# mattayes/tigerbeetle

Measured on AMD Instinct MI355X. Metric: transfers/sec committed (whole node, bit-exact results) + p99 batch latency, higher is better.
Workload: dtype u128

## Files before the change

### tigerbeetle_amd/csrc/engine.hip

```cpp
#include <hip/hip_runtime.h>

#include <algorithm>
#include <atomic>
#include <chrono>
#include <cmath>
#include <cstdarg>
#include <cstdio>
#include <cstdlib>
#include <cstring>
#include <numeric>
#include <string>
#include <vector>
#include <map>
#include <functional>
#include <mutex>

#include "../../include/tbgpu.h"
#include "../../include/tbgpu_bench.h"
#include "../../include/tbgpu_shard.h"
#include "k_apply.h"
#include "k_flow.h"
#include "k_aux.h"
#include "k_replay.h"
#include "k_route.h"
// ... 306 lines not shown
    u64* h_rmeta = nullptr;
};

static inline BalView ckpt_view(const tbgpu* E) {
    return BalView{E->ckpt_bal, E->ckpt_bal ? E->ckpt_bal + 4 * E->account_cap : nullptr};
}

static void ckpt_note_ids(tbgpu* E, const u8* records, u64 n);

static int api_enter(tbgpu* E, bool mutates) {
    E->pf_input = nullptr;
    E->api_calls++;
    if (mutates && E->poisoned) {
        return fail(TBGPU_STATUS_PANIC, "engine stopped by an earlier device panic (tbgpu_reset or tbgpu_deinit it)");
    }
    return TBGPU_STATUS_OK;
}
#define API_ENTER(E, mutates)                        \
    do {                                             \
        if (const int st_ = api_enter((E), (mutates))) return st_; \
    } while (0)

static u64 pipe_reply_bytes(const tbgpu* E) { return 16 + E->meta_cap * 4 + (u64)E->pe_max * 8; }

#define PROF_EVENTS 8192

static int prof_begin(tbgpu* E, ProfilePair* p, int kind) {
    p->kind = -1;
    if (!E->profile || !(E->prof_mask & (1u << kind))) return 0;
    if (E->event_next + 2 > E->event_pool.size()) return 0;
    p->kind = kind;
    p->a = E->event_pool[E->event_next++];
    p->b = E->event_pool[E->event_next++];
    HIPCK(hipEventRecord(p->a, E->stream));
    return 0;
}

static int prof_end(tbgpu* E, ProfilePair* p) {
    if (!E->profile || p->kind < 0) return 0;
    HIPCK(hipEventRecord(p->b, E->stream));
    E->prof.push_back(*p);
    return 0;
}

static int prof_collect(tbgpu* E) {
    if (!E->kclock_used.empty()) {
        HIPCK(hipMemcpy(E->h_kclock, E->kclock, (u64)E->kclock_next * KCLOCK_WORDS * 8, hipMemcpyDeviceToHost));
        for (const auto& u : E->kclock_used) {
            const u64* w = E->h_kclock + (u64)u.first * KCLOCK_WORDS;
            for (u32 k = 0; k < 3; k++) {
                const u64* kw = w + k * KCLOCK_STRIDE;
                u64 end = 0;
                for (u32 q = 1; q <= KCLOCK_ENDS; q++) end = std::max(end, kw[q * KCLOCK_LINE]);
                if (k == 0) end = w[KCLOCK_STRIDE];
                if (!((u.second >> k) & 1) || end < kw[0] || !E->wall_khz) continue;
                E->span_ms[k] += (double)(end - kw[0]) / E->wall_khz;
                E->span_n[k] += 1;
            }
        }
        E->kclock_used.clear();
        E->kclock_next = 0;
    }
    for (const ProfilePair& p : E->prof) {
        float ms = 0;
        HIPCK(hipEventElapsedTime(&ms, p.a, p.b));
        E->prof_ms[p.kind] += ms;
        E->prof_n[p.kind] += 1;
        if (p.kind == K_PASS) E->pass_ms.push_back(ms);
    }
    E->prof.clear();
    E->event_next = 0;
    return 0;
}


static int engine_clear(tbgpu* E) {
    HIPCK(hipMemsetAsync(E->T.acct_hot, 0, E->account_cap * sizeof(AccountHot), E->stream));
    HIPCK(hipMemsetAsync(E->T.bal.lo, 0, E->account_cap * sizeof(AccountBal), E->stream));
    HIPCK(hipMemsetAsync(E->T.acct_cold, 0, E->account_cap * sizeof(AccountCold), E->stream));
    HIPCK(hipMemsetAsync(E->T.account_mark, 0, E->account_cap * sizeof(u32), E->stream));
    HIPCK(hipMemsetAsync(E->T.xidx, 0, E->xidx_cap * sizeof(u64), E->stream));
    HIPCK(hipMemsetAsync(E->T.xdup, 0, E->xidx_cap, E->stream));
    HIPCK(hipMemsetAsync(E->T.xposted, 0, E->xlog_cap, E->stream));
    HIPCK(hipMemsetAsync(E->bloom, 0, (E->bloom_mask + 1) / 8, E->stream));
    E->log_next = 0;
    E->evicted_total = 0;
    HIPCK(hipMemsetAsync(E->g, 0, sizeof(Globals), E->stream));
    HIPCK(hipStreamSynchronize(E->stream));
    E->epoch = 0;
    E->dedup_force = true;
    E->commit_ts = 0;
    E->last_batch_ts = 0;
    E->pending = false;
    E->balances_set = false;
    return TBGPU_STATUS_OK;
}

static std::mutex g_dev_mu;
static std::map<int, u32> g_dev_engines;

static void dev_register(tbgpu* E, bool add) {
    std::lock_guard<std::mutex> lock(g_dev_mu);
    if (add && !E->dev_registered) {
        g_dev_engines[E->device]++;
        E->dev_registered = true;
    } else if (!add && E->dev_registered) {
        if (--g_dev_engines[E->device] == 0) g_dev_engines.erase(E->device);
        E->dev_registered = false;
    }
}

__global__ __launch_bounds__(FLOW_THREADS) void tb_residency_probe(u32* counter, u32 total, u64 deadline, u32* failed) {
    extern __shared__ u32 s_probe_lds[];
    if (threadIdx.x != 0) return;
    s_probe_lds[0] = 0;
    atomicAdd(counter, 1u);
    const u64 t0 = wall_clock64();
    while (__hip_atomic_load(counter, __ATOMIC_RELAXED, __HIP_MEMORY_SCOPE_AGENT) < total) {
        if (wall_clock64() - t0 > deadline) {
            atomicOr(failed, 1u);
            return;
        }
        __builtin_amdgcn_s_sleep(8);
    }
}

static int residency_probe(tbgpu* E, u32 grid) {
    Owner scratch;
    u32* d = nullptr;
    HIPCK(tbMalloc(scratch, &d, 8));
    hipFuncAttributes attr{};
    size_t lds = 0;
    if (hipFuncGetAttributes(&attr, reinterpret_cast<const void*>(&tb_flow)) == hipSuccess) lds = attr.sharedSizeBytes;
    lds = std::max<size_t>(lds, 4);
    int probe_occ = 0;
    if (E->flow_occ &&
        hipOccupancyMaxActiveBlocksPerMultiprocessor(&probe_occ, reinterpret_cast<const void*>(&tb_residency_probe),
                                                     FLOW_THREADS, lds) == hipSuccess &&
        probe_occ > (int)E->flow_occ) {
        grid = (u32)(((u64)grid * (u64)probe_occ + E->flow_occ - 1) / E->flow_occ);
    }
    int st = TBGPU_STATUS_OK;
    u32 h[2] = {0, 0};
    hipError_t e = hipMemsetAsync(d, 0, 8, E->stream);
    if (e == hipSuccess) {
        hipLaunchKernelGGL(tb_residency_probe, dim3(grid), dim3(FLOW_THREADS), std::max<size_t>(lds, 4), E->stream, d, grid,
                           (u64)200 * E->wall_khz, d + 1);
        e = hipGetLastError();
    }
    if (e == hipSuccess) e = hipMemcpyAsync(h, d, 8, hipMemcpyDeviceToHost, E->stream);
    if (e == hipSuccess) e = hipStreamSynchronize(E->stream);
    if (e != hipSuccess) return fail(TBGPU_STATUS_DEVICE, "tbgpu_init: residency probe: %s", hipGetErrorString(e));
    if (h[1]) {
        st = fail(TBGPU_STATUS_DEVICE,
                  "tbgpu_init: device %d is not exclusive: %u workgroups of the ordered fallback's grid could not be "
                  "resident together (another process or kernel holds its CUs; tbgpu.h \"Device exclusivity\")",
                  E->device, grid);
    }
    return st;
}

static u32 flow_grid(tbgpu* E) {
    u32 engines = 1;
    {
        std::lock_guard<std::mutex> lock(g_dev_mu);
        auto it = g_dev_engines.find(E->device);
// ... 23 lines not shown
                                     tbgpu_delta_counts* counts);
static int node_api_get_stats(TbNode* N, tbgpu_stats* s);
static void node_reset_stats(TbNode* N);
static u32 node_world(TbNode* N);
static tbgpu* node_engine(TbNode* N, u32 d);
static int node_api_imports(TbNode* N, u32 d, u64 out[3]);
static int node_api_register_host(TbNode* N, void* ptr, u64 bytes);
static int node_api_unregister_host(TbNode* N, void* ptr);
static int node_fetch(TbNode* N, bool accounts, const u64* ids, u32 n, u8* out, u8* found);
static int node_api_accounts_in(TbNode* N, const void* records, u32 n, bool load);
static int node_api_transfers_in(TbNode* N, const void* records, const u8* state, u32 n, bool load);
static int node_api_set_commit_timestamp(TbNode* N, u64 timestamp);
static int query_init(tbgpu* E);
static void query_free(tbgpu* E);

static int engine_init(tbgpu* E);

extern "C" int tbgpu_init(const tbgpu_config* config, tbgpu_t** out) {
    *out = nullptr;
    if (config && config->device_count > 1) return node_api_init(config, out);
    if (!config || config->accounts_max == 0 || config->transfers_max == 0 || config->pass_events_max == 0 ||
        config->pass_batches_max == 0) {
        return fail(TBGPU_STATUS_INVALID, "tbgpu_init: invalid config");
    }
    if (config->accounts_max > (1ULL << 31) || config->transfers_max > (1ULL << 31)) {
        return fail(TBGPU_STATUS_INVALID, "tbgpu_init: table capacity above 2^31 objects per device");
    }
    int ndev = 0;
    if (hipGetDeviceCount(&ndev) != hipSuccess || ndev == 0) {
        return fail(TBGPU_STATUS_DEVICE, "tbgpu_init: no HIP device visible");
    }
    if (config->device < 0 || config->device >= ndev) {
        return fail(TBGPU_STATUS_INVALID, "tbgpu_init: device %d out of range (%d devices)", config->device, ndev);
    }
    tbgpu* E = new tbgpu();
    E->cfg = *config;
    E->device = config->device;
    E->profile = (config->flags & TBGPU_CONFIG_PROFILE) != 0;
#ifdef TBGPU_TIMING_KNOBS
    if (const char* ab = getenv("TBGPU_ABLATE")) E->ablate = (u32)strtoul(ab, nullptr, 0);
    E->kclock_off = getenv("TBGPU_NO_KCLOCK") != nullptr;
#endif
    const int st = engine_init(E);
    if (st) {
        tbgpu_deinit(E);
        return st;
    }
    *out = E;
    return TBGPU_STATUS_OK;
}

static int engine_init(tbgpu* E) {
    const tbgpu_config* config = &E->cfg;
    HIPCK(hipSetDevice(E->device));
    HIPCK(tbStreamCreate(E->own, &E->stream));
    dev_register(E, true);

    u64 load = 2;
#ifdef TBGPU_TIMING_KNOBS
    if (const char* s = getenv("TBGPU_ACCOUNT_SLOTS")) load = std::max<u64>(2, strtoull(s, nullptr, 0));
#endif
    E->account_cap = pow2_at_least(std::max<u64>(load * config->accounts_max, 1024));
    E->xlog_cap = std::max<u64>(config->transfers_max, 1024);
    E->xidx_cap = pow2_at_least(std::max<u64>(2 * E->xlog_cap, 2048));
    E->pe_max = config->pass_events_max;
    E->pb_max = config->pass_batches_max;
    if (const char* v = getenv("TBGPU_NO_LEAN")) E->lean_ok = atoi(v) == 0;
    if (const char* v = getenv("TBGPU_WB_BOUND")) E->wb_bound_ok = atoi(v) != 0;
    if (const char* v = getenv("TBGPU_WB_STAGE")) E->wb_stage = atoi(v) != 0;
    E->dedup_cap = pow2_at_least(std::max<u64>(4ULL * E->pe_max, 64));
    E->undo_cap = 4 * (BATCH_EVENTS_MAX + 1);
    E->meta_cap = std::max<u64>(E->pb_max, 1 << 16);
    E->lookup_cap = 1 << 16;
    {
        u32 shift = 0;
        while ((E->account_cap >> shift) > LEG_BUCKETS_PREF && (1u << shift) < LEG_SLOTS_MAX) shift++;
        E->leg_shift = shift;
        E->leg_buckets = (u32)(E->account_cap >> shift);
        E->legs_ok = E->leg_buckets <= LEG_BUCKETS_MAX;
    }

    size_t free_b = 0, total_b = 0;
    HIPCK(hipMemGetInfo(&free_b, &total_b));
    const u64 need = E->account_cap * (sizeof(Account) + 4) + E->xlog_cap * (sizeof(Transfer) + 1) +
                     E->xidx_cap * (sizeof(u64) + 1) +
                     (u64)E->pe_max * (4 * 4 + 8 * 4 + 128 * PIPE_SLOTS + 8 + 4) + E->dedup_cap * 8;
    if (need > free_b) {
        return fail(TBGPU_STATUS_INVALID, "tbgpu_init: needs %llu bytes of HBM, %llu free",
                    (unsigned long long)need, (unsigned long long)free_b);
    }

    HIPCK(tbMalloc(E->own, &E->T.acct_hot, E->account_cap * sizeof(AccountHot)));
    HIPCK(tbMalloc(E->own, &E->T.bal.lo, E->account_cap * sizeof(AccountBal)));
    E->T.bal.hi = E->T.bal.lo + 4 * E->account_cap;
    HIPCK(tbMalloc(E->own, &E->T.acct_cold, E->account_cap * sizeof(AccountCold)));
    HIPCK(tbMalloc(E->own, &E->T.account_mark, E->account_cap * sizeof(u32)));
    HIPCK(tbMalloc(E->own, &E->T.xidx, E->xidx_cap * sizeof(u64)));
    HIPCK(tbMalloc(E->own, &E->T.xdup, E->xidx_cap));
    HIPCK(tbMalloc(E->own, &E->T.xlog, E->xlog_cap * sizeof(Transfer)));
    HIPCK(tbMalloc(E->own, &E->T.xposted, E->xlog_cap));
    HIPCK(tbMalloc(E->own, &E->g, sizeof(Globals)));
    {
        const u64 bits = std::min<u64>(1ULL << 34, pow2_at_least(std::max<u64>(1ULL << 16, 8 * E->xlog_cap)));
        E->bloom_mask = bits - 1;
        HIPCK(tbMalloc(E->own, &E->bloom, bits / 8));
    }
    {
        hipDeviceProp_t prop;
        int occ = 0;
        if (hipGetDeviceProperties(&prop, E->device) == hipSuccess &&
            hipOccupancyMaxActiveBlocksPerMultiprocessor(&occ, reinterpret_cast<const void*>(&tb_flow), FLOW_THREADS, 0) ==
                hipSuccess &&
            occ >= 1) {
            E->F.grid = (u32)std::max(1, std::min(prop.multiProcessorCount / 4, 64));
#ifdef TBGPU_TIMING_KNOBS
            if (const char* gs = getenv("TBGPU_FLOW_GRID")) E->F.grid = std::max(1u, std::min(E->F.grid, (u32)atoi(gs)));
#endif
            E->flow_capacity = (u64)occ * prop.multiProcessorCount;
            E->flow_occ = (u32)occ;
            E->F.grid = (u32)std::min<u64>(E->F.grid, E->flow_capacity);
            E->F.grid_alloc = E->F.grid;
            int khz = 0;
            if (hipDeviceGetAttribute(&khz, hipDeviceAttributeWallClockRate, E->device) != hipSuccess) khz = 0;
            khz = std::max(khz, 100000);
            E->F.stall_ticks = 60ULL * 1000ULL * (u64)khz;
            if (const char* ms = getenv("TBGPU_STALL_MS")) {
                E->F.stall_ticks = std::max<u64>(1, strtoull(ms, nullptr, 10)) * (u64)khz;
            }
            E->wall_khz = (u64)khz;
            if (getenv("TBGPU_DEBUG")) {
                fprintf(stderr, "tbgpu: flow grid %u, occupancy %d, wall clock %d kHz, stall ticks %llu\n", E->F.grid,
                        occ, khz, (unsigned long long)E->F.stall_ticks);
            }
            E->flow_ok = E->pb_max <= FLOW_NB_MAX && !(config->flags & TBGPU_CONFIG_SEQUENTIAL_FALLBACK);
#ifdef TBGPU_TIMING_KNOBS
            if (getenv("TBGPU_NO_FLOW")) E->flow_ok = false;
#endif
        }
    }
    E->T.account_mask = E->account_cap - 1;
    E->T.xidx_mask = E->xidx_cap - 1;
    E->T.xlog_cap = E->xlog_cap;
    E->T.g = E->g;

    const u64 pe = E->pe_max;
    HIPCK(tbMalloc(E->own, &E->info, pe * 4));
    HIPCK(tbMalloc(E->own, &E->eflags, pe * 2));
    HIPCK(tbMalloc(E->own, &E->dr, pe * 4));
    HIPCK(tbMalloc(E->own, &E->cr, pe * 4));
    HIPCK(tbMalloc(E->own, &E->ps, pe * 4));
    HIPCK(tbMalloc(E->own, &E->rs, pe * 4));
    HIPCK(tbMalloc(E->own, &E->dep_list, pe * 4));
    HIPCK(tbMalloc(E->own, &E->dep_count, (u64)E->pb_max * 4));
    HIPCK(tbMalloc(E->own, &E->amt, pe * 16));
    HIPCK(tbMalloc(E->own, &E->kid, pe * 8));
    HIPCK(tbMalloc(E->own, &E->kpid, pe * 8));
    HIPCK(tbMalloc(E->own, &E->dedup, E->dedup_cap * 8));
    HIPCK(tbMalloc(E->own, &E->sum_shards, SUM_WORDS * 8));
    HIPCK(tbMalloc(E->own, &E->undo, (u64)E->undo_cap * sizeof(UndoEntry)));
    if (E->legs_ok) {
        HIPCK(tbMalloc(E->own, &E->resolve_slow, (u64)E->pb_max * 4));
        HIPCK(tbMalloc(E->own, &E->leg_w, pe * 2 * 8));
        HIPCK(tbMalloc(E->own, &E->leg_off, (u64)std::min<u32>(E->pb_max, LEG_PREPARES_MAX) * (E->leg_buckets + 1) * 4));
        HIPCK(tbMalloc(E->own, &E->leg_tot, ((u64)E->leg_buckets + 1) * 4));
        HIPCK(hipMemset(E->leg_tot, 0, ((u64)E->leg_buckets + 1) * 4));
    }
    if (E->flow_ok) {
        FlowArgs& F = E->F;
        HIPCK(tbMalloc(E->own, &F.f_pe, pe * 4));
        HIPCK(tbMalloc(E->own, &F.f_batch, pe * 4));
        HIPCK(tbMalloc(E->own, &F.f_len, pe * 4));
        HIPCK(tbMalloc(E->own, &F.need, pe * 4));
        HIPCK(tbMalloc(E->own, &F.nsucc, pe * 4));
        HIPCK(tbMalloc(E->own, &F.queue, pe * 4));
        HIPCK(tbMalloc(E->own, &F.uflags, pe * 4));
        HIPCK(tbMalloc(E->own, &F.nacct, pe * 4));
        HIPCK(tbMalloc(E->own, &F.rpos, pe * 4));
        HIPCK(tbMalloc(E->own, &F.succ, pe * 4 * FLOW_RMAX));
        HIPCK(tbMalloc(E->own, &F.run, pe * sizeof(RunEntry) * FLOW_RMAX));
        for (int k = 0; k < 2; k++) {
            HIPCK(tbMalloc(E->own, &F.keys[k], pe * 4 * FLOW_RMAX));
            HIPCK(tbMalloc(E->own, &F.vals[k], pe * 4 * FLOW_RMAX));
        }
// ... 2178 lines not shown
extern "C" int tbgpu_load_accounts(tbgpu_t* E, const void* records, uint32_t n) {
    API_ENTER(E, true);
    if (E->node) return node_api_accounts_in(E->node, records, n, true);
    return upsert_accounts(E, records, n, true);
}

static int upsert_transfers(tbgpu* E, const void* records, const uint8_t* state, uint32_t n, bool if_absent) {
    HIPCK(hipSetDevice(E->device));
    if (if_absent) {
        if (E->pending) {
            int st = engine_sync(E);
            if (st) return st;
        }
        int st = load_snapshot(E, records, n);
        if (st) return st;
    }
    if (E->pending) {
        int st = engine_sync(E);
        if (st) return st;
    }
    HIPCK(hipMemsetAsync(E->d_status, 0, 8, E->stream));
    for (u32 c = 0; c < n; c += E->lookup_cap) {
        const u32 m = std::min<u32>(E->lookup_cap, n - c);
        HIPCK(hipMemcpyAsync(E->lookup_out, (const u8*)records + (u64)c * 128, (u64)m * 128, hipMemcpyHostToDevice,
                             E->stream));
        HIPCK(hipMemcpyAsync(E->lookup_found, state + c, m, hipMemcpyHostToDevice, E->stream));
        HIPCK(hipMemsetAsync(E->d_status + 1, 0, 4, E->stream));
        hipLaunchKernelGGL(tb_upsert_transfers, dim3((m + 255) / 256), dim3(256), 0, E->stream, E->T, E->lookup_out,
                           E->lookup_found, m, E->log_next, E->d_status + 1, E->d_status, if_absent ? 1u : 0u,
                           nullptr);
        HIPCK(hipGetLastError());
        u32 added = 0;
        HIPCK(hipMemcpyAsync(&added, E->d_status + 1, 4, hipMemcpyDeviceToHost, E->stream));
        HIPCK(hipStreamSynchronize(E->stream));
        E->log_next += added;
    }
    u32 status = 0;
    HIPCK(hipMemcpy(&status, E->d_status, 4, hipMemcpyDeviceToHost));
    if (status) return fail(TBGPU_STATUS_PANIC, "transfer log or index full");
    return TBGPU_STATUS_OK;
}

extern "C" int tbgpu_upsert_transfers(tbgpu_t* E, const void* records, const uint8_t* state, uint32_t n) {
    API_ENTER(E, true);
    if (E->node) return node_api_transfers_in(E->node, records, state, n, false);
    return upsert_transfers(E, records, state, n, false);
}

extern "C" int tbgpu_load_transfers(tbgpu_t* E, const void* records, const uint8_t* posted_state, uint32_t n) {
    API_ENTER(E, true);
    if (E->node) return node_api_transfers_in(E->node, records, posted_state, n, true);
    std::vector<u8> st(n);
    for (u32 i = 0; i < n; i++) {
        if (posted_state[i] > POSTED_VOIDED) return fail(TBGPU_STATUS_INVALID, "posted state %u", posted_state[i]);
        st[i] = (u8)(posted_state[i] + 1);
    }
    return upsert_transfers(E, records, st.data(), n, true);
}

static int engine_evict(tbgpu_t* E, uint64_t keep, uint64_t* evicted) {
    *evicted = 0;
    HIPCK(hipSetDevice(E->device));
    if (E->wb.inflight) return fail(TBGPU_STATUS_INVALID, "an asynchronous write-back is in flight");
    int st = engine_sync(E);
    if (st) return st;
    if (E->ckpt_valid && E->ckpt_pos != E->log_next)
        return fail(TBGPU_STATUS_INVALID, "%llu log positions written since the last write-back",
                    (unsigned long long)(E->log_next - E->ckpt_pos));
    const u64 written = E->ckpt_valid ? E->ckpt_pos : 0;
    const u64 cut = std::min<u64>(written, E->log_next > keep ? E->log_next - keep : 0);
    if (cut == 0) return TBGPU_STATUS_OK;
    const u64 n = E->log_next, kept = n - cut;
    u8* live = E->T.xdup;
    u64* d_evicted = E->wb.d_cnt;
    HIPCK(hipMemsetAsync(d_evicted, 0, 8, E->stream));
    const u32 grid = (u32)std::min<u64>(4096, std::max<u64>(1, (n + 255) / 256));
    hipLaunchKernelGGL(tb_evict_scan, dim3(grid), dim3(256), 0, E->stream, E->T, cut, n, E->bloom, E->bloom_mask, live,
                       d_evicted);
    HIPCK(hipGetLastError());
    for (u64 a = 0; a < kept; a += cut) {
        const u64 m = std::min<u64>(cut, kept - a);
        HIPCK(hipMemcpyAsync(E->T.xlog + a, E->T.xlog + cut + a, m * sizeof(Transfer), hipMemcpyDeviceToDevice, E->stream));
        HIPCK(hipMemcpyAsync(E->T.xposted + a, E->T.xposted + cut + a, m, hipMemcpyDeviceToDevice, E->stream));
    }
    HIPCK(hipMemsetAsync(E->T.xlog + kept, 0, cut * sizeof(Transfer), E->stream));
    HIPCK(hipMemsetAsync(E->T.xposted + kept, 0, cut, E->stream));
    HIPCK(hipMemsetAsync(E->T.xidx, 0, E->xidx_cap * sizeof(u64), E->stream));
    if (kept) {
        hipLaunchKernelGGL(tb_evict_reindex, dim3((u32)std::min<u64>(4096, (kept + 255) / 256)), dim3(256), 0, E->stream,
                           E->T, kept, (const u8*)live);
        HIPCK(hipGetLastError());
    }
    HIPCK(hipMemsetAsync(E->T.xdup, 0, E->xidx_cap, E->stream));
    u64 h_evicted = 0;
    HIPCK(hipMemcpyAsync(&h_evicted, d_evicted, 8, hipMemcpyDeviceToHost, E->stream));
    HIPCK(hipStreamSynchronize(E->stream));
    E->log_next = kept;
    E->ckpt_pos -= cut;
    E->evicted_total += h_evicted;
    E->dedup_force = true;
    if (h_evicted) {
        HIPCK(hipMemcpy(E->h_globals, E->g, sizeof(Globals), hipMemcpyDeviceToHost));
        E->h_globals->transfer_count -= std::min<u64>(E->h_globals->transfer_count, h_evicted);
        HIPCK(hipMemcpy(&E->g->transfer_count, &E->h_globals->transfer_count, 8, hipMemcpyHostToDevice));
    }
    *evicted = h_evicted;
    return TBGPU_STATUS_OK;
}


extern "C" int tbgpu_evict_transfers(tbgpu_t* E, uint64_t keep, uint64_t* evicted) {
    API_ENTER(E, true);
    *evicted = 0;
    if (E->node) return node_api_evict(E->node, keep, evicted);
    return engine_evict(E, keep, evicted);
}

static int engine_maybe_cold(tbgpu_t* E, const uint64_t* ids, uint32_t n, uint8_t* cold) {
    if (n == 0) return TBGPU_STATUS_OK;
    if (E->evicted_total == 0) {
        memset(cold, 0, n);
        return TBGPU_STATUS_OK;
    }
    HIPCK(hipSetDevice(E->device));
    if (E->pending) {
        const int st = engine_sync(E);
        if (st) return st;
    }
    for (u32 i0 = 0; i0 < n; i0 += E->lookup_cap) {
        const u32 m = std::min<u32>(n - i0, E->lookup_cap);
        HIPCK(hipMemcpyAsync(E->lookup_ids, ids + 2 * (u64)i0, (u64)m * 16, hipMemcpyHostToDevice, E->stream));
        hipLaunchKernelGGL(tb_cold_query, dim3((m + 255) / 256), dim3(256), 0, E->stream, E->T, (const u64*)E->bloom,
                           E->bloom_mask, E->lookup_ids, m, E->lookup_found);
        HIPCK(hipGetLastError());
        HIPCK(hipMemcpyAsync(cold + i0, E->lookup_found, m, hipMemcpyDeviceToHost, E->stream));
        HIPCK(hipStreamSynchronize(E->stream));
    }
    return TBGPU_STATUS_OK;
}

extern "C" int tbgpu_transfers_maybe_cold(tbgpu_t* E, const uint64_t* ids, uint32_t n, uint8_t* cold) {
    API_ENTER(E, false);
    if (E->node) return node_api_maybe_cold(E->node, ids, n, cold);
    return engine_maybe_cold(E, ids, n, cold);
}

extern "C" int tbgpu_set_commit_timestamp(tbgpu_t* E, uint64_t timestamp) {
    API_ENTER(E, true);
    if (E->node) return node_api_set_commit_timestamp(E->node, timestamp);
    HIPCK(hipSetDevice(E->device));
    if (E->pending) {
        int st = engine_sync(E);
        if (st) return st;
    }
    E->commit_ts = timestamp;
    E->last_batch_ts = timestamp;
    HIPCK(hipMemcpyAsync(&E->g->commit_timestamp, &E->commit_ts, 8, hipMemcpyHostToDevice, E->stream));
    HIPCK(hipStreamSynchronize(E->stream));
    return TBGPU_STATUS_OK;
}

#include "query.h"
#include "node.h"
```

### tigerbeetle_amd/csrc/k_aux.h

```cpp
#pragma once

#include "pass.h"

template <bool ACCOUNTS>
__global__ void tb_lookup(Tables T, const u64* ids, u32 n, u8* out, u8* found) {
    const u32 i = blockIdx.x * blockDim.x + threadIdx.x;
    if (i >= n) return;
    const u64 lo = ids[2 * i], hi = ids[2 * i + 1];
    if (ACCOUNTS) {
        const u32 slot = tb_account_find(T, lo, hi);
        found[i] = slot != TB_NOT_FOUND;
        if (slot != TB_NOT_FOUND) *(Account*)(out + (u64)i * 128) = tb_account_load(T, slot);
    } else {
        const u32 pos = tb_transfer_find(T, lo, hi);
        found[i] = pos != TB_NOT_FOUND;
        if (pos != TB_NOT_FOUND) *(Transfer*)(out + (u64)i * 128) = T.xlog[pos];
    }
}

__global__ void tb_export_accounts(Tables T, u64 first, u64 cap, u8* out, u64* count) {
    const u64 i = first + (u64)blockIdx.x * blockDim.x + threadIdx.x;
    if (i >= cap) return;
    const AccountHot& h = T.acct_hot[i];
    if (h.timestamp == 0 || tb_id_reserved(h.id_lo, h.id_hi)) return;
    const u64 k = atomicAdd((unsigned long long*)count, 1ULL);
    *(Account*)(out + k * 128) = tb_account_load(T, (u32)i);
}

__global__ void tb_export_transfers(Tables T, u64 first, u64 n, u8* out, u64* count, u64* posted_out,
                                    u64* posted_count) {
    const u64 i = first + (u64)blockIdx.x * blockDim.x + threadIdx.x;
    if (i >= first + n) return;
    const u64 e = T.xidx[i];
    if (e == 0 || (e & XI_TOMB)) return;
    const u32 pos = tb_xi_pos(e);
    const Transfer& t = T.xlog[pos];
    const u64 k = atomicAdd((unsigned long long*)count, 1ULL);
    *(Transfer*)(out + k * 128) = t;
    const u8 st = T.xposted[pos];
    if (st != POSTED_NONE) {
        const u64 q = atomicAdd((unsigned long long*)posted_count, 1ULL);
        posted_out[2 * q] = t.timestamp;
        posted_out[2 * q + 1] = st == POSTED_POSTED ? 0 : 1;
    }
}

__global__ void tb_set_balances(Tables T, u64 lo, u64 hi, u64 dp_lo, u64 dp_hi, u64 dpo_lo, u64 dpo_hi,
                                u64 cp_lo, u64 cp_hi, u64 cpo_lo, u64 cpo_hi, u32* status) {
    const u32 slot = tb_account_find(T, lo, hi);
    if (slot == TB_NOT_FOUND) {
        *status = 1;
        return;
    }
    AccountBal a;
    a.debits_pending = tb_u128(dp_lo, dp_hi);
    a.debits_posted = tb_u128(dpo_lo, dpo_hi);
    a.credits_pending = tb_u128(cp_lo, cp_hi);
    a.credits_posted = tb_u128(cpo_lo, cpo_hi);
    tb_bal_store(T.bal, slot, a);
    const u128 d = tb_sat_add(a.debits_pending, a.debits_posted);
    const u128 c = tb_sat_add(a.credits_pending, a.credits_posted);
    u128 bound = tb_u128(T.g->bound_lo, T.g->bound_hi);
    if (d > bound) bound = d;
    if (c > bound) bound = c;
    T.g->bound_lo = tb_lo(bound);
    T.g->bound_hi = tb_hi(bound);
    *status = 0;
}

__global__ void tb_zero_balances(Tables T, u64 cap) {
    const u64 i = (u64)blockIdx.x * blockDim.x + threadIdx.x;
    if (i == 0) {
        T.g->transfer_count = 0;
        T.g->bound_lo = 0;
        T.g->bound_hi = 0;
    }
    if (i >= cap) return;
    tb_bal_store(T.bal, i, AccountBal{0, 0, 0, 0});
}

__global__ void tb_delta_accounts(Tables T, BalView snap, u64 ts0, u64 first, u64 last, u8* out, u64 cap,
                                  u64* count, AccountBal* before, u32 world, u32 self) {
    const u64 i = first + (u64)blockIdx.x * blockDim.x + threadIdx.x;
    if (i >= last) return;
    const AccountHot& h = T.acct_hot[i];
    if (h.timestamp == 0 || tb_id_reserved(h.id_lo, h.id_hi)) return;
    if (world > 1 && tb_home(h.id_lo, h.id_hi, world) != self) return;
    const AccountBal b = tb_bal_load(T.bal, i), s = tb_bal_load(snap, i);
    const bool same = b.debits_pending == s.debits_pending && b.debits_posted == s.debits_posted &&
                      b.credits_pending == s.credits_pending && b.credits_posted == s.credits_posted;
    if (h.timestamp <= ts0 && same) return;
    const u64 k = atomicAdd((unsigned long long*)count, 1ULL);
    if (k < cap) {
        *(Account*)(out + k * 128) = tb_account_load(T, (u32)i);
        if (before) before[k] = h.timestamp <= ts0 ? s : AccountBal{0, 0, 0, 0};
    }
}

#define DELTA_THREADS 256

__device__ static inline bool tb_delta_live(const Tables& T, u64 pos, u64 ts0) {
    const Transfer& t = T.xlog[pos];
    return t.timestamp > ts0 && tb_transfer_find(T, tb_lo(t.id), tb_hi(t.id)) == (u32)pos;
}

__global__ __launch_bounds__(DELTA_THREADS) void tb_delta_log_count(Tables T, u64 pos0, u64 n, u64 ts0, u32* block_counts) {
    __shared__ u32 s_wave[DELTA_THREADS / 64];
    const u64 i = (u64)blockIdx.x * DELTA_THREADS + threadIdx.x;
    const bool live = i < n && tb_delta_live(T, pos0 + i, ts0);
    const u64 m = __ballot(live);
    if ((threadIdx.x & 63) == 0) s_wave[threadIdx.x >> 6] = __popcll(m);
    __syncthreads();
    if (threadIdx.x == 0) {
        u32 c = 0;
        for (u32 w = 0; w < DELTA_THREADS / 64; w++) c += s_wave[w];
        block_counts[blockIdx.x] = c;
    }
}

__global__ __launch_bounds__(DELTA_THREADS) void tb_delta_log_scatter(Tables T, u64 pos0, u64 n, u64 ts0, const u64* block_base,
                                                                      u8* out, u64* ids, u64* pv, u64* pv_count) {
    __shared__ u32 s_wave[DELTA_THREADS / 64];
    const u64 i = (u64)blockIdx.x * DELTA_THREADS + threadIdx.x;
    const bool live = i < n && tb_delta_live(T, pos0 + i, ts0);
    const u64 m = __ballot(live);
    const u32 lane = threadIdx.x & 63, wave = threadIdx.x >> 6;
    if (lane == 0) s_wave[wave] = __popcll(m);
    __syncthreads();
    if (!live) return;
    u64 k = block_base[blockIdx.x] + __popcll(m & ((1ULL << lane) - 1));
    for (u32 w = 0; w < wave; w++) k += s_wave[w];
    const Transfer& t = T.xlog[pos0 + i];
    if (out) *(Transfer*)(out + k * 128) = t;
    if (ids) {
        ids[4 * k] = tb_lo(t.debit_account_id);
        ids[4 * k + 1] = tb_hi(t.debit_account_id);
        ids[4 * k + 2] = tb_lo(t.credit_account_id);
        ids[4 * k + 3] = tb_hi(t.credit_account_id);
    }
    if (pv && (t.flags & (TF_POST | TF_VOID))) {
        const u64 q = atomicAdd((unsigned long long*)pv_count, 1ULL);
        pv[3 * q] = tb_lo(t.pending_id);
        pv[3 * q + 1] = tb_hi(t.pending_id);
        pv[3 * q + 2] = (t.flags & TF_POST) ? 0 : 1;
    }
}

__global__ __launch_bounds__(1024) void tb_delta_scan_blocks(const u32* counts, u64 nblocks, u64* base, u64* total) {
    __shared__ u32 s_wave[1024 / 64];
    const u64 per = (nblocks + 1023) / 1024;
    const u64 k0 = min(nblocks, (u64)threadIdx.x * per), k1 = min(nblocks, k0 + per);
    u32 local = 0;
    for (u64 k = k0; k < k1; k++) local += counts[k];
    u32 all;
    u64 run = tb_block_excl_sum(local, s_wave, &all);
    for (u64 k = k0; k < k1; k++) {
        base[k] = run;
        run += counts[k];
    }
    if (threadIdx.x == 0) *total = all;
}

__global__ void tb_delta_posted(Tables T, const u64* pv, const u64* npv, u64* pairs, u64* status) {
    const u64 q = (u64)blockIdx.x * blockDim.x + threadIdx.x;
    if (q >= *npv) return;
    const u32 pos = tb_transfer_find(T, pv[3 * q], pv[3 * q + 1]);
    if (pos == TB_NOT_FOUND) {
        atomicOr((unsigned long long*)status, 1ULL);
        return;
    }
    pairs[2 * q] = T.xlog[pos].timestamp;
    pairs[2 * q + 1] = pv[3 * q + 2];
}

__global__ __launch_bounds__(256) void tb_delta_ids(Tables T, BalView snap, u64 ts0, const u64* ids, u64 n,
                                                    u32* mark, u32 epoch, u8* out, AccountBal* before, u64* count,
                                                    u32* slots, u64* slot_count, const u64* n_dev = nullptr) {
    const u64 i = (u64)blockIdx.x * blockDim.x + threadIdx.x;
    const bool live = i < n && !(n_dev && i >= 2 * *n_dev);
    u32 slot = TB_NOT_FOUND;
    if (live) slot = tb_account_find(T, ids[2 * i], ids[2 * i + 1]);
    u32 was = epoch;
    AccountHot h{};
    AccountBal b{}, sn{};
    AccountCold c{};
    if (slot != TB_NOT_FOUND) {
        was = atomicExch(&mark[slot], epoch);
        h = T.acct_hot[slot];
        b = tb_bal_load(T.bal, slot);
        sn = tb_bal_load(snap, slot);
        c = T.acct_cold[slot];
    }
    const bool first = was != epoch;
    const bool same = b.debits_pending == sn.debits_pending && b.debits_posted == sn.debits_posted &&
                      b.credits_pending == sn.credits_pending && b.credits_posted == sn.credits_posted;
    const bool emit = first && (h.timestamp > ts0 || !same);
    const u64 si = tb_wave_claim(first, slot_count);
    if (first) slots[si] = slot;
    const u64 k = tb_wave_claim(emit, count);
    if (emit) {
        Account a;
        a.id = tb_u128(h.id_lo, h.id_hi);
        a.debits_pending = b.debits_pending;
        a.debits_posted = b.debits_posted;
        a.credits_pending = b.credits_pending;
        a.credits_posted = b.credits_posted;
        a.user_data_128 = c.user_data_128;
        a.user_data_64 = c.user_data_64;
        a.user_data_32 = c.user_data_32;
        a.reserved = c.reserved;
        a.ledger = h.ledger;
        a.code = h.code;
        a.flags = h.flags;
        a.timestamp = h.timestamp;
        *(Account*)(out + k * 128) = a;
        before[k] = h.timestamp <= ts0 ? sn : AccountBal{0, 0, 0, 0};
    }
}

__global__ __launch_bounds__(256) void tb_delta_capture(Tables T, const u64* ids, u64 n, u32* mark, u32 epoch,
                                                        u32* slots, AccountBal* cap, u64* slot_count,
                                                        const u64* n_dev = nullptr) {
    const u64 i = (u64)blockIdx.x * blockDim.x + threadIdx.x;
    const bool live = i < n && !(n_dev && i >= 2 * *n_dev);
    u32 slot = TB_NOT_FOUND;
    if (live) slot = tb_account_find(T, ids[2 * i], ids[2 * i + 1]);
    u32 was = epoch;
    AccountBal b{};
    if (slot != TB_NOT_FOUND) {
        was = atomicExch(&mark[slot], epoch);
        b = tb_bal_load(T.bal, slot);
    }
    const bool first = was != epoch;
    const u64 si = tb_wave_claim(first, slot_count);
    if (first) {
        slots[si] = slot;
        cap[si] = b;
    }
}

__global__ __launch_bounds__(256) void tb_delta_capture_log(Tables T, u64 pos0, u64 n, u32* mark, u32 epoch, u32* slots,
                                                            AccountBal* cap, u64* slot_count) {
    const u64 i = (u64)blockIdx.x * blockDim.x + threadIdx.x;
    u32 ds = TB_NOT_FOUND, cs = TB_NOT_FOUND;
    if (i < n) {
        const u64* w = (const u64*)&T.xlog[pos0 + i];
        const u64 dlo = w[2], dhi = w[3], clo = w[4], chi = w[5];
        if (!tb_id_reserved(dlo, dhi) && !tb_id_reserved(clo, chi)) {
            const u64 dpos = tb_hash_id(dlo, dhi) & T.account_mask, cpos = tb_hash_id(clo, chi) & T.account_mask;
            const AccountHot d0 = T.acct_hot[dpos], c0 = T.acct_hot[cpos];
            AccountHot dh, ch;
            tb_account_find2(T, dlo, dhi, dpos, d0, clo, chi, cpos, c0, &ds, &cs, &dh, &ch);
        } else {
            if (!tb_id_reserved(dlo, dhi)) ds = tb_account_find(T, dlo, dhi);
// ... 135 lines not shown
```

### tigerbeetle_amd/csrc/k_change_events.h

```cpp
#pragma once

#include "k_balances.h"

#define CHANGE_EVENTS_MAX 2730u
#define CHANGE_ACCOUNTS_MAX (2 * CHANGE_EVENTS_MAX)
#define CHANGE_SET_SLOTS_MAX 16384u
#define CHANGE_SET_SLOTS_MIN 256u
#define CHANGE_LDS_BINS 512u
#define CHANGE_LDS_BINS_SLOTS_MAX 8192u
#define CHANGE_NONE 0xFFFFFFFFu
#define CHANGE_THREADS 512
#define CHANGE_TILES 16
#define CHANGE_FLAG_ORPHAN 0

__host__ __device__ static inline u64 tb_change_hash(u64 lo, u64 hi) { return tb_mix64(tb_hash_id(lo, hi) ^ 0x9e3779b97f4a7c15ULL); }
__host__ __device__ static inline u32 tb_change_entry(u64 h, u32 index) { return (u32)(h >> 48) << 16 | (index + 1); }

__host__ static inline u32 tb_change_lds_bins(u32 slots) { return slots <= CHANGE_LDS_BINS_SLOTS_MAX ? CHANGE_LDS_BINS : 0; }
__host__ static inline u32 tb_change_set_slots(u32 accounts) {
    u32 s = CHANGE_SET_SLOTS_MIN;
    while (s < 2 * accounts) s <<= 1;
    return s;
}

// ... 11 lines not shown
        s = (s + 1) & mask;
    }
    return CHANGE_NONE;
}

__device__ static inline u32 tb_change_probe(const u16* s_set, u32 mask, const u64* ids, u64 lo, u64 hi) {
    const u64 h = tb_change_hash(lo, hi);
    const u32 tag = (u32)(h >> 61);
    u32 s = (u32)h & mask;
    for (u32 i = 0; i <= mask; i++) {
        const u32 e = s_set[s];
        if (e == 0) return CHANGE_NONE;
        if ((e >> 13) == tag) {
            const u32 index = (e & 0x1FFFu) - 1;
            if (ids[2 * (u64)index] == lo && ids[2 * (u64)index + 1] == hi) return index;
        }
        s = (s + 1) & mask;
    }
    return CHANGE_NONE;
}

template <typename ENTRY>
__device__ static inline ENTRY tb_change_lds_entry(u32 e) {
    if (sizeof(ENTRY) == 4) return (ENTRY)e;
    return (ENTRY)(e ? (e >> 29) << 13 | (e & 0x1FFFu) : 0);
}

__device__ static inline u32 tb_change_bin_claim(u32* tags, u32 bins, u32 index) {
    u32 s = index % bins;
#pragma unroll
    for (u32 k = 0; k < 2; k++) {
        const u32 old = atomicCAS(&tags[s], CHANGE_NONE, index);
        if (old == CHANGE_NONE || old == index) return s;
        s = ((index * 0x9E3779B1u) >> 7) % bins;
    }
    return CHANGE_NONE;
}

__device__ static inline u128 tb_shfl128(u128 v, u32 from) {
    const u64 lo = __shfl((unsigned long long)tb_lo(v), (int)from);
    const u64 hi = __shfl((unsigned long long)tb_hi(v), (int)from);
    return tb_u128(lo, hi);
}

__global__ __launch_bounds__(QUERY_THREADS) void tb_change_gather(NodeTablesArgs N, const u64* ids, u32 n_accounts, u8* accounts,
                                                                  u32* found, const u64* pids, u32 n_rows, u64* P, u32* found_p) {
    const u32 i = blockIdx.x * QUERY_THREADS + threadIdx.x;
    if (i < n_accounts) {
        const u64 lo = ids[2 * (u64)i], hi = ids[2 * (u64)i + 1];
        const Tables& O = N.T[tb_home(lo, hi, N.world)];
        const u32 slot = tb_account_find(O, lo, hi);
        found[i] = slot != TB_NOT_FOUND;
        if (slot != TB_NOT_FOUND) *(Account*)(accounts + (u64)i * 128) = tb_account_load(O, slot);
    }
    if (i < n_rows) {
        u128 p = 0;
        found_p[i] = tb_pending_amount(N, pids[2 * (u64)i], pids[2 * (u64)i + 1], &p);
        P[2 * (u64)i] = tb_lo(p), P[2 * (u64)i + 1] = tb_hi(p);
    }
}

template <typename ENTRY, bool CACHED>
__global__ __launch_bounds__(CHANGE_THREADS) void tb_change_effects(NodeTablesArgs N, u32 self, u64 n, u64 t_last, const u32* set,
                                                                   u32 mask, const u64* ids, u32 n_accounts, u64* bins,
                                                                   u32 lds_bins_max) {
    extern __shared__ __attribute__((aligned(16))) u8 s_lds[];
    ENTRY* s_set = (ENTRY*)s_lds;
    u64* s_bins = (u64*)(s_set + mask + 1);
    const Tables& T = N.T[self];
    const u32 lane = threadIdx.x & 63;
    u64* flags = bins + (u64)n_accounts * BALANCE_SLOT_WORDS;
    const u32 lds_bins = CACHED || n_accounts >= lds_bins_max ? lds_bins_max : n_accounts;
    u32* s_tags = (u32*)(s_bins + lds_bins * BALANCE_SLOT_WORDS);
    for (u32 i = threadIdx.x; i <= mask; i += CHANGE_THREADS) s_set[i] = tb_change_lds_entry<ENTRY>(set[i]);
    for (u32 i = threadIdx.x; i < lds_bins * BALANCE_SLOT_WORDS; i += CHANGE_THREADS) s_bins[i] = 0;
    if (CACHED) {
        for (u32 i = threadIdx.x; i < lds_bins; i += CHANGE_THREADS) s_tags[i] = CHANGE_NONE;
    }
    __syncthreads();
    for (u32 t = 0; t < CHANGE_TILES; t++) {
        const u64 tile0 = ((u64)blockIdx.x * CHANGE_TILES + t) * CHANGE_THREADS, pos = tile0 + threadIdx.x;
        if (tile0 >= n) break;
        const u64* w = (const u64*)&T.xlog[pos < n ? pos : 0];
        const u64 ts = pos < n ? w[15] : 0;
        const bool newer = ts > t_last;
        if (__ballot(newer) == 0) continue;
        u32 idx[2] = {CHANGE_NONE, CHANGE_NONE};
        u128 pend = 0, post = 0;
        if (newer) {
            const ulonglong2 d = ((const ulonglong2*)w)[1], c = ((const ulonglong2*)w)[2];
            idx[0] = tb_change_probe(s_set, mask, ids, d.x, d.y);
            idx[1] = tb_change_probe(s_set, mask, ids, c.x, c.y);
        }
        if ((idx[0] & idx[1]) != CHANGE_NONE) {
            const u64 lo = w[0], hi = w[1];
            if (tb_id_reserved(lo, hi) || tb_transfer_find(T, lo, hi) != (u32)pos) {
                idx[0] = idx[1] = CHANGE_NONE;
            } else {
                const u128 amount = tb_u128(w[6], w[7]);
                const u32 tf = (u32)(w[14] >> 48);
                u128 p = amount;
                if (tb_effect_is_post(tf) && !tb_pending_amount(N, w[8], w[9], &p)) {
                    atomicOr((unsigned long long*)(flags + CHANGE_FLAG_ORPHAN), 1ULL);
                }
                const BalanceEffect e = tb_balance_effect(tf, amount, p);
                pend = e.pend, post = e.post;
            }
        }
#pragma unroll
        for (u32 side = 0; side < 2; side++) {
            const u32 my = idx[side];
            bool adds = my != CHANGE_NONE;
            u128 v0 = adds ? pend : (u128)0, v1 = adds ? post : (u128)0;
            u32 nxt = lane;
            bool chains = false;
            u64 todo = __ballot(adds);
            while (todo) {
                const int leader = __ffsll((unsigned long long)todo) - 1;
                const u32 b = __shfl(my, leader);
                const bool mine = my == b;
                const u64 group = __ballot(mine);
                todo &= ~group;
                if ((group & (group - 1)) == 0) continue;
                chains = true;
                if (mine) {
                    const u64 above = lane == 63 ? 0 : group & ~((2ULL << lane) - 1);
                    if (above) nxt = (u32)__ffsll((unsigned long long)above) - 1;
                    if ((int)lane != leader) adds = false;
                }
            }
            if (chains) {
#pragma unroll
                for (u32 s = 0; s < 6; s++) {
                    const bool has = nxt != lane;
                    const u128 o0 = tb_shfl128(v0, nxt), o1 = tb_shfl128(v1, nxt);
                    const u32 nn = __shfl(nxt, nxt);
                    if (has) {
                        v0 += o0, v1 += o1;
                        nxt = nn == nxt ? lane : nn;
                    }
                }
            }
            u32 at = my;
            if (CACHED && adds) at = tb_change_bin_claim(s_tags, lds_bins, my);
            if (adds && at < lds_bins) {
                u64* dst = s_bins + at * BALANCE_SLOT_WORDS + 4 * side;
                tb_atomic_add128(dst, v0);
                tb_atomic_add128(dst + 2, v1);
            } else if (adds) {
                u64* dst = bins + (u64)my * BALANCE_SLOT_WORDS + 4 * side;
                tb_atomic_add128(dst, v0);
                tb_atomic_add128(dst + 2, v1);
            }
        }
    }
    __syncthreads();
    for (u32 i = threadIdx.x; i < lds_bins * 4; i += CHANGE_THREADS) {
        const u32 index = CACHED ? s_tags[i >> 2] : i >> 2;
        if (CACHED && index == CHANGE_NONE) continue;
        tb_atomic_add128(bins + (u64)index * BALANCE_SLOT_WORDS + 2 * (i & 3), tb_u128(s_bins[2 * i], s_bins[2 * i + 1]));
    }
}
```

### tigerbeetle_amd/csrc/k_evict.h

```cpp
#pragma once

#include "pass.h"

#define BLOOM_K 3

__host__ __device__ static inline u64 tb_bloom_bit(u64 lo, u64 hi, u32 k, u64 mask) {
    return tb_mix64(tb_fingerprint(lo, hi) + 0x9e3779b97f4a7c15ULL * (k + 1)) & mask;
}

__device__ static inline void tb_bloom_add(u64* bits, u64 mask, u64 lo, u64 hi) {
#pragma unroll
    for (u32 k = 0; k < BLOOM_K; k++) {
        const u64 b = tb_bloom_bit(lo, hi, k, mask);
        atomicOr((unsigned long long*)&bits[b >> 6], 1ULL << (b & 63));
    }
}

__device__ static inline bool tb_bloom_maybe(const u64* bits, u64 mask, u64 lo, u64 hi) {
#pragma unroll
    for (u32 k = 0; k < BLOOM_K; k++) {
        const u64 b = tb_bloom_bit(lo, hi, k, mask);
        if (!((bits[b >> 6] >> (b & 63)) & 1)) return false;
    }
    return true;
}

__global__ void tb_evict_scan(Tables T, u64 cut, u64 n, u64* bloom, u64 mask, u8* live, u64* evicted) {
    u64 mine = 0;
    for (u64 pos = (u64)blockIdx.x * blockDim.x + threadIdx.x; pos < n; pos += (u64)gridDim.x * blockDim.x) {
        const Transfer& t = T.xlog[pos];
        const u64 lo = tb_lo(t.id), hi = tb_hi(t.id);
        const bool alive = t.timestamp != 0 && !tb_id_reserved(lo, hi) && tb_transfer_find(T, lo, hi) == (u32)pos;
        if (pos < cut) {
            if (alive) {
                tb_bloom_add(bloom, mask, lo, hi);
                mine++;
            }
        } else {
            live[pos - cut] = alive ? 1 : 0;
        }
    }
    for (int off = 32; off > 0; off >>= 1) mine += __shfl_xor((unsigned long long)mine, off);
    if ((threadIdx.x & 63) == 0 && mine) atomicAdd((unsigned long long*)evicted, (unsigned long long)mine);
}

__global__ void tb_evict_reindex(Tables T, u64 n, const u8* live) {
    for (u64 pos = (u64)blockIdx.x * blockDim.x + threadIdx.x; pos < n; pos += (u64)gridDim.x * blockDim.x) {
        if (!live[pos]) continue;
        const Transfer& t = T.xlog[pos];
        (void)tb_transfer_claim_new(T, tb_lo(t.id), tb_hi(t.id), (u32)pos);
    }
}

__global__ void tb_cold_query(Tables T, const u64* bloom, u64 mask, const u64* ids, u32 n, u8* out) {
    const u32 i = blockIdx.x * blockDim.x + threadIdx.x;
    if (i >= n) return;
    const u64 lo = ids[2 * i], hi = ids[2 * i + 1];
    out[i] = !tb_id_reserved(lo, hi) && tb_transfer_find(T, lo, hi) == TB_NOT_FOUND && tb_bloom_maybe(bloom, mask, lo, hi);
}
```

### tigerbeetle_amd/csrc/k_ledgers.h

```cpp
#pragma once

#include "k_change_events.h"

#define LEDGERS_MAX 1024u
#define LEDGER_SET_SLOTS_MIN 64u
#define LEDGER_SET_SLOTS_MAX (2 * LEDGERS_MAX)
#define LEDGER_THREADS 512
#define LEDGER_LOG_TILES 16
#define LEDGER_TABLE_TILES 4
#define LEDGER_LDS_BINS 256u
#define LEDGER_BIN_WORDS 16
#define LEDGER_BIN_COUNT 8
#define LEDGER_BIN_EFFECTS 10
#define LEDGER_BINS(slots) ((u64)(slots) + 2)
#define LEDGER_TABLE_WORDS 10
#define LEDGER_LOG_WORDS 4

__host__ static inline u32 tb_ledger_set_slots(u32 ledgers) {
    u32 s = LEDGER_SET_SLOTS_MIN;
    while (s < 2 * ledgers) s <<= 1;
    return s;
}
__host__ __device__ static inline u32 tb_ledger_hash(u32 ledger) { return (u32)(tb_mix64(ledger) >> 32); }

// ... 73 lines not shown
                                                                      const u32* set, u32 mask, u32 all, u64* bins) {
    extern __shared__ __attribute__((aligned(16))) u8 s_lds[];
    u32* s_set = (u32*)s_lds;
    u64* s_bins = (u64*)(s_set + mask + 1);
    u64* s_all = s_bins + LEDGER_LDS_BINS * LEDGER_TABLE_WORDS;
    u32* s_tags = (u32*)(s_all + LEDGER_TABLE_WORDS);
    const u32 lane = threadIdx.x & 63;
    for (u32 i = threadIdx.x; i <= mask; i += LEDGER_THREADS) s_set[i] = set[i];
    for (u32 i = threadIdx.x; i < (LEDGER_LDS_BINS + 1) * LEDGER_TABLE_WORDS; i += LEDGER_THREADS) s_bins[i] = 0;
    for (u32 i = threadIdx.x; i < LEDGER_LDS_BINS; i += LEDGER_THREADS) s_tags[i] = CHANGE_NONE;
    __syncthreads();
    u128 held[4] = {0, 0, 0, 0};
    u32 held_count = 0;
    for (u32 t = 0; t < LEDGER_TABLE_TILES; t++) {
        const u64 tile0 = ((u64)blockIdx.x * LEDGER_TABLE_TILES + t) * LEDGER_THREADS, slot = tile0 + threadIdx.x;
        if (tile0 >= cap) break;
        bool live = false;
        u32 ledger = 0;
        u64 ts = 0;
        if (slot < cap) {
            const ulonglong2* e = (const ulonglong2*)&T.acct_hot[slot];
            const ulonglong2 id = e[0], r = e[1];
            ledger = (u32)r.x, ts = r.y;
            live = ts != 0 && !tb_id_reserved(id.x, id.y) && tb_home(id.x, id.y, world) == self;
        }
        if (__ballot(live) == 0) continue;
        const u32 my = live ? tb_ledger_probe(s_set, mask, ledger) : CHANGE_NONE;
        bool adds = my != CHANGE_NONE;
        u128 v[4] = {0, 0, 0, 0};
        u32 count = 0;
        if (live && (adds || all)) {
            const AccountBal b = tb_bal_load(T.bal, slot);
            v[0] = b.debits_pending, v[1] = b.debits_posted, v[2] = b.credits_pending, v[3] = b.credits_posted;
            count = t_at == 0 || ts <= t_at;
        }
        if (all) {
#pragma unroll
            for (u32 c = 0; c < 4; c++) held[c] += tb_wave_sum128(v[c]);
            held_count += (u32)__popcll(__ballot(count != 0));
        }
        if (__ballot(adds) == 0) continue;
        tb_ledger_combine<4>(lane, my, adds, v, count);
        if (adds) {
            u64* dst = bins + (u64)my * LEDGER_BIN_WORDS;
            tb_ledger_add<4, LEDGER_TABLE_WORDS>(s_tags, s_bins, my, v, count, dst, dst + LEDGER_BIN_COUNT);
        }
    }
    if (all && lane == 0) {
#pragma unroll
        for (u32 c = 0; c < 4; c++) tb_atomic_add128(s_all + 2 * c, held[c]);
        if (held_count) atomicAdd((unsigned long long*)(s_all + 8), (unsigned long long)held_count);
    }
    __syncthreads();
    for (u32 i = threadIdx.x; i < (LEDGER_LDS_BINS + 1) * 5; i += LEDGER_THREADS) {
        const u32 b = i / 5, c = i % 5;
        const u32 index = b == LEDGER_LDS_BINS ? mask + 1 : s_tags[b];
        if (index == CHANGE_NONE) continue;
        const u64* src = s_bins + b * LEDGER_TABLE_WORDS + 2 * c;
        u64* dst = bins + (u64)index * LEDGER_BIN_WORDS + 2 * c;
        if (c < 4) tb_atomic_add128(dst, tb_u128(src[0], src[1]));
        else if (src[0]) atomicAdd((unsigned long long*)dst, (unsigned long long)src[0]);
    }
}

__global__ __launch_bounds__(LEDGER_THREADS) void tb_ledger_effects(NodeTablesArgs N, u32 self, u64 n, u64 t_at, const u32* set,
                                                                     u32 mask, u32 all, u64* bins) {
    extern __shared__ __attribute__((aligned(16))) u8 s_lds[];
    u32* s_set = (u32*)s_lds;
    u64* s_bins = (u64*)(s_set + mask + 1);
    u64* s_all = s_bins + LEDGER_LDS_BINS * LEDGER_LOG_WORDS;
    u32* s_tags = (u32*)(s_all + LEDGER_LOG_WORDS);
    const Tables& T = N.T[self];
    const u32 lane = threadIdx.x & 63;
    u64* flags = bins + ((u64)mask + 2) * LEDGER_BIN_WORDS;
    for (u32 i = threadIdx.x; i <= mask; i += LEDGER_THREADS) s_set[i] = set[i];
    for (u32 i = threadIdx.x; i < (LEDGER_LDS_BINS + 1) * LEDGER_LOG_WORDS; i += LEDGER_THREADS) s_bins[i] = 0;
    for (u32 i = threadIdx.x; i < LEDGER_LDS_BINS; i += LEDGER_THREADS) s_tags[i] = CHANGE_NONE;
    __syncthreads();
    u128 held[2] = {0, 0};
    for (u32 t = 0; t < LEDGER_LOG_TILES; t++) {
        const u64 tile0 = ((u64)blockIdx.x * LEDGER_LOG_TILES + t) * LEDGER_THREADS, pos = tile0 + threadIdx.x;
        if (tile0 >= n) break;
        const u64* w = (const u64*)&T.xlog[pos < n ? pos : 0];
        const u64 ts = pos < n ? w[15] : 0;
        const bool newer = ts > t_at;
        if (__ballot(newer) == 0) continue;
        u32 my = CHANGE_NONE;
        u64 tail = 0;
        if (newer) {
            tail = w[14];
            my = tb_ledger_probe(s_set, mask, (u32)tail);
        }
        bool adds = my != CHANGE_NONE;
        u128 v[2] = {0, 0};
        bool sums = false;
        if (newer && (adds || all)) {
            const u64 lo = w[0], hi = w[1];
            if (!tb_id_reserved(lo, hi) && tb_transfer_find(T, lo, hi) == (u32)pos) {
                const u128 amount = tb_u128(w[6], w[7]);
                const u32 tf = (u32)(tail >> 48);
                u128 p = amount;
                if (tb_effect_is_post(tf) && !tb_pending_amount(N, w[8], w[9], &p)) {
                    atomicOr((unsigned long long*)(flags + CHANGE_FLAG_ORPHAN), 1ULL);
                }
                const BalanceEffect e = tb_balance_effect(tf, amount, p);
                v[0] = e.pend, v[1] = e.post;
                sums = true;
            }
        }
        adds = adds && sums;
        if (all) held[0] += tb_wave_sum128(v[0]), held[1] += tb_wave_sum128(v[1]);
        if (__ballot(adds) == 0) continue;
        u32 none = 0;
        tb_ledger_combine<2>(lane, my, adds, v, none);
        if (adds) {
            u64* dst = bins + (u64)my * LEDGER_BIN_WORDS + LEDGER_BIN_EFFECTS;
            tb_ledger_add<2, LEDGER_LOG_WORDS>(s_tags, s_bins, my, v, 0, dst, dst);
        }
    }
    if (all && lane == 0) tb_atomic_add128(s_all, held[0]), tb_atomic_add128(s_all + 2, held[1]);
    __syncthreads();
    for (u32 i = threadIdx.x; i < (LEDGER_LDS_BINS + 1) * 2; i += LEDGER_THREADS) {
        const u32 b = i >> 1, c = i & 1;
        const u32 index = b == LEDGER_LDS_BINS ? mask + 1 : s_tags[b];
        if (index == CHANGE_NONE) continue;
        const u64* src = s_bins + b * LEDGER_LOG_WORDS + 2 * c;
        tb_atomic_add128(bins + (u64)index * LEDGER_BIN_WORDS + LEDGER_BIN_EFFECTS + 2 * c, tb_u128(src[0], src[1]));
    }
}
```

### tigerbeetle_amd/csrc/k_node.h

```cpp
#pragma once

#include "k_route.h"

#define NODE_WORLD_MAX 16

struct NodeGatherArgs {
    const u8* src[NODE_WORLD_MAX];
    u64 start[NODE_WORLD_MAX + 1];
    u32 world;
    u8* recv;
};

#define GATHER_PER 4
__global__ __launch_bounds__(256) void tb_node_gather(NodeGatherArgs A) {
    const u64 n8 = A.start[A.world] * 8;
    const u64 base = (u64)blockIdx.x * 256 * GATHER_PER + threadIdx.x;
    u32x4 v[GATHER_PER];
#pragma unroll
    for (u32 q = 0; q < GATHER_PER; q++) {
        const u64 idx = base + q * 256;
        if (idx >= n8) continue;
        const u64 i = idx >> 3;
        u32 s = 0;
        while (s + 1 < A.world && A.start[s + 1] <= i) s++;
// ... 571 lines not shown
        s = tb_seq_source(A, g);
        e = g - A.start[s];
        d = A.dep[s][e] != 0;
    }
    const u32 lane = threadIdx.x & 63, wave = threadIdx.x >> 6;
    const u64 m = __ballot(d);
    if (lane == 0) s_wave[wave] = (u32)__popcll(m);
    __syncthreads();
    u32 before = 0;
    for (u32 w = 0; w < wave; w++) before += s_wave[w];
    if (!live) return;
    if (!d) {
        A.map[g] = 0xFFFFFFFFu;
        return;
    }
    const u32 r = A.blk[blockIdx.x] + before + (u32)__popcll(m & ((1ULL << lane) - 1));
    A.map[g] = r;
    const u64* off = A.meta[s];
    const u32 b = tb_batch_search(off, 0, A.nb[s], e);
    const u64 L = off[b + 1] - off[b];
    A.out_ts[r] = off[A.nb[s] + 1 + b] - L + 1 + (e - off[b]);
    const u32x4* in = (const u32x4*)(A.src[s] + e * 128);
    u32x4 v[8];
#pragma unroll
    for (u32 k = 0; k < 8; k++) v[k] = in[k];
    u32x4* dst = (u32x4*)(A.out + (u64)r * 128);
#pragma unroll
    for (u32 k = 0; k < 8; k++) dst[k] = v[k];
    const u64* w = (const u64*)v;
    tb_seq_insert(tset, w[0], w[1]);
    if (((const u16*)v)[59] & (TF_POST | TF_VOID)) tb_seq_insert(tset, w[8], w[9]);
}

__global__ void tb_seq_meta(SeqCompactArgs A) {
    const u32 nbp = A.pstart[A.world];
    for (u32 k = blockIdx.x * blockDim.x + threadIdx.x; k <= nbp; k += gridDim.x * blockDim.x) {
        u64 g;
        u64 ts = 0;
        if (k == nbp) {
            g = A.start[A.world];
        } else {
            u32 s = 0;
            while (s + 1 < A.world && A.pstart[s + 1] <= k) s++;
            const u32 b = k - A.pstart[s];
            g = A.start[s] + A.meta[s][b];
            ts = A.meta[s][A.nb[s] + 1 + b];
        }
        const u64 blk = g >> 8;
        u32 r = A.blk[blk];
        for (u64 q = blk << 8; q < g; q++) {
            const u32 s = tb_seq_source(A, q);
            r += A.dep[s][q - A.start[s]] != 0;
        }
        A.xmeta[k] = r;
        if (k < nbp) A.xmeta[nbp + 1 + k] = ts;
    }
}

__global__ void tb_seq_expand(SeqCompactArgs A, const u8* xcodes, u8* codes) {
    const u64 n = A.start[A.world];
    for (u64 g = (u64)blockIdx.x * blockDim.x + threadIdx.x; g < n; g += (u64)gridDim.x * blockDim.x) {
        const u32 r = A.map[g];
        if (r != 0xFFFFFFFFu) codes[g] = xcodes[r];
    }
}

__global__ void tb_seq_fold(const Globals* xg, Globals* g0, u64 bound0_lo, u64 bound0_hi) {
    if (blockIdx.x || threadIdx.x) return;
    g0->panic |= xg->panic;
    if (xg->commit_timestamp > g0->commit_timestamp) g0->commit_timestamp = xg->commit_timestamp;
    const u128 grow = tb_u128(xg->bound_lo, xg->bound_hi) - tb_u128(bound0_lo, bound0_hi);
    const u128 b = tb_sat_add(tb_u128(g0->bound_lo, g0->bound_hi), grow);
    g0->bound_lo = tb_lo(b);
    g0->bound_hi = tb_hi(b);
}

__global__ void tb_seq_load_transfers(NodeTablesArgs N, SeqSet tset, Tables X, u64* loaded, SeqSet aset) {
    const u64 n = tset.count[0];
    for (u64 i = (u64)blockIdx.x * blockDim.x + threadIdx.x; i < n; i += (u64)gridDim.x * blockDim.x) {
        SeqEntry& q = tset.e[tset.list[i]];
        const Tables& H = N.T[tb_home(q.lo, q.hi, N.world)];
        const u32 pos = tb_transfer_find(H, q.lo, q.hi);
        if (pos == TB_NOT_FOUND) continue;
        const Transfer t = H.xlog[pos];
        const u32 xp = (u32)tb_wave_claim(true, loaded);
        X.xlog[xp] = t;
        X.xposted[xp] = H.xposted[pos];
        q.x = xp;
        q.home = pos;
        if (tb_transfer_claim_new(X, q.lo, q.hi, xp) == TB_NOT_FOUND) continue;
        tb_seq_insert(aset, tb_lo(t.debit_account_id), tb_hi(t.debit_account_id));
        tb_seq_insert(aset, tb_lo(t.credit_account_id), tb_hi(t.credit_account_id));
    }
}

__global__ __launch_bounds__(256) void tb_seq_event_accounts(const u8* events, u64 n, SeqSet aset) {
    __shared__ WgDedup s_d;
    tb_wg_dedup_reset(s_d);
    const u64 g = (u64)blockIdx.x * 256 + threadIdx.x;
    const bool live = g < n && !(((const u16*)(events + g * 128))[59] & 0x8000);
    u64 lo[2] = {0, 0}, hi[2] = {0, 0};
    u32 st[2];
#pragma unroll
    for (u32 s = 0; s < 2; s++) {
        if (live) {
            const u64* w = (const u64*)(events + g * 128) + 2 + 2 * s;
            lo[s] = w[0];
            hi[s] = w[1];
        }
        st[s] = tb_wg_dedup_claim(s_d, live && !tb_id_reserved(lo[s], hi[s]), lo[s], hi[s]);
    }
    __syncthreads();
#pragma unroll
    for (u32 s = 0; s < 2; s++) {
        if (tb_wg_dedup_go(s_d, st[s], lo[s], hi[s])) tb_seq_insert(aset, lo[s], hi[s]);
    }
}

__global__ void tb_seq_load_accounts(NodeTablesArgs N, SeqSet aset, Tables X, AccountBal* bal0) {
    const u64 n = aset.count[0];
    for (u64 i = (u64)blockIdx.x * blockDim.x + threadIdx.x; i < n; i += (u64)gridDim.x * blockDim.x) {
        SeqEntry& q = aset.e[aset.list[i]];
        const Tables& O = N.T[tb_home(q.lo, q.hi, N.world)];
        const u32 os = tb_account_find(O, q.lo, q.hi);
        if (os == TB_NOT_FOUND) continue;
        const Account a = tb_account_load(O, os);
        if (bal0) {
            AccountBal b;
            b.debits_pending = a.debits_pending;
            b.debits_posted = a.debits_posted;
            b.credits_pending = a.credits_pending;
            b.credits_posted = a.credits_posted;
            bal0[i] = b;
        }
        const u32 xs = tb_account_claim(X, q.lo, q.hi, a.timestamp);
        if (xs == TB_NOT_FOUND) continue;
        tb_account_store_new(X, xs, a);
        q.x = xs;
        q.home = os;
    }
}

__global__ void tb_seq_writeback_transfers(Tables X, u64 base, u64 n, SeqSet tset, Tables H, u32 self, u32 world,
                                           u64 h_base, u64* h_count) {
    const u64 stride = (u64)gridDim.x * blockDim.x;
    for (u64 i = (u64)blockIdx.x * blockDim.x + threadIdx.x; i < n; i += stride) {
        const Transfer& t = X.xlog[base + i];
        if (t.timestamp == 0 || tb_home(tb_lo(t.id), tb_hi(t.id), world) != self) continue;
        if (tb_transfer_find(X, tb_lo(t.id), tb_hi(t.id)) != (u32)(base + i)) continue;
        const u64 lp = h_base + tb_wave_claim(true, h_count);
        if (lp >= H.xlog_cap) {
            tb_panic(H.g, PANIC_TABLE_FULL);
            continue;
        }
        H.xlog[lp] = t;
        H.xposted[lp] = X.xposted[base + i];
        if (tb_transfer_claim_new(H, tb_lo(t.id), tb_hi(t.id), (u32)lp) == TB_NOT_FOUND) continue;
        (void)tb_wave_claim(true, &H.g->transfer_count);
    }
    const u64 m = tset.count[0];
    for (u64 i = (u64)blockIdx.x * blockDim.x + threadIdx.x; i < m; i += stride) {
        const SeqEntry& q = tset.e[tset.list[i]];
        if (q.x == TB_NOT_FOUND || tb_home(q.lo, q.hi, world) != self) continue;
        const u8 st = X.xposted[q.x];
        if (H.xposted[q.home] != st) H.xposted[q.home] = st;
    }
}

__global__ void tb_seq_writeback_accounts(Tables X, SeqSet aset, Tables O, u32 self, u32 world, const AccountBal* bal0) {
    const u64 n = aset.count[0];
    for (u64 i = (u64)blockIdx.x * blockDim.x + threadIdx.x; i < n; i += (u64)gridDim.x * blockDim.x) {
        const SeqEntry& q = aset.e[aset.list[i]];
        if (q.x == TB_NOT_FOUND || q.home == SEQ_NEW || tb_home(q.lo, q.hi, world) != self) continue;
        const AccountBal x = tb_bal_load(X.bal, q.x), b = bal0[i];
        if (x.debits_pending != b.debits_pending) tb_bal_add(O.bal, q.home, BAL_DP, x.debits_pending - b.debits_pending);
        if (x.debits_posted != b.debits_posted) tb_bal_add(O.bal, q.home, BAL_DPOST, x.debits_posted - b.debits_posted);
        if (x.credits_pending != b.credits_pending) tb_bal_add(O.bal, q.home, BAL_CP, x.credits_pending - b.credits_pending);
        if (x.credits_posted != b.credits_posted) tb_bal_add(O.bal, q.home, BAL_CPOST, x.credits_posted - b.credits_posted);
    }
}

__global__ __launch_bounds__(256) void tb_seq_account_ids(const u8* events, u64 n, SeqSet aset) {
    const u64 g = (u64)blockIdx.x * 256 + threadIdx.x;
    if (g >= n) return;
    const u64* w = (const u64*)(events + g * 128);
    tb_seq_insert(aset, w[0], w[1]);
}

__global__ void tb_seq_locate_new(SeqSet aset, Tables X) {
    const u64 n = aset.count[0];
    for (u64 i = (u64)blockIdx.x * blockDim.x + threadIdx.x; i < n; i += (u64)gridDim.x * blockDim.x) {
        SeqEntry& q = aset.e[aset.list[i]];
        if (q.x != TB_NOT_FOUND) continue;
        const u32 xs = tb_account_find(X, q.lo, q.hi);
        if (xs == TB_NOT_FOUND) continue;
        q.x = xs;
        q.home = SEQ_NEW;
    }
}

__global__ void tb_seq_writeback_new_accounts(Tables X, SeqSet aset, Tables O, u32 self, u32 world, u64* limbits,
                                              u64 limmask) {
    const u64 n = aset.count[0];
    for (u64 i = (u64)blockIdx.x * blockDim.x + threadIdx.x; i < n; i += (u64)gridDim.x * blockDim.x) {
        const SeqEntry& q = aset.e[aset.list[i]];
        if (q.home != SEQ_NEW) continue;
        const Account a = tb_account_load(X, q.x);
        if (a.flags & AF_LIMITS) tb_limit_set(limbits, limmask, q.lo, q.hi);
        if (tb_home(q.lo, q.hi, world) != self) continue;
        const u32 slot = tb_account_claim(O, q.lo, q.hi, a.timestamp);
        if (slot == TB_NOT_FOUND) continue;
        tb_account_store_new(O, slot, a);
        (void)tb_wave_claim(true, &O.g->account_count);
    }
}

__global__ void tb_seq_xidx_list(Tables X, const u64* loaded, const u8* events, u64 base, u64 n, u32* list, u64* count,
                                 u64 cap) {
    const u64 L = *loaded, total = L + n;
    for (u64 i = (u64)blockIdx.x * blockDim.x + threadIdx.x; i < total; i += (u64)gridDim.x * blockDim.x) {
        u64 lo, hi, pos;
        if (i < L) {
            lo = tb_lo(X.xlog[i].id);
            hi = tb_hi(X.xlog[i].id);
            pos = i;
        } else {
            const u64* w = (const u64*)(events + (i - L) * 128);
            lo = w[0];
            hi = w[1];
            pos = base + (i - L);
// ... 50 lines not shown
```

### tigerbeetle_amd/csrc/k_pending.h

```cpp
#pragma once

#include "k_change_events.h"

#define PENDING_ROWS_MAX 4095u
#define PENDING_THREADS 256
#define PENDING_TILES 16

__global__ __launch_bounds__(QUERY_THREADS) void tb_pending_gather(Tables T, QueryPendingFilter flt, const u64* positions, u32 m,
                                                                   u64 n, u8* out) {
    const u32 i = blockIdx.x * QUERY_THREADS + threadIdx.x;
    if (i >= m) return;
    const u64 pos = positions[i];
    if (pos >= n) return;
    const ulonglong2* c = (const ulonglong2*)&T.xlog[pos];
    const ulonglong2 b = c[6], d = c[7];
    const QueryPendingFields f{d.y, (u32)(b.y >> 32), (u32)(d.x >> 48)};
    *(Transfer*)(out + (u64)i * 128) = T.xlog[pos];
    flt.states[i] = (u8)flt.state(f, T.xposted, pos);
}

__global__ __launch_bounds__(PENDING_THREADS) void tb_pending_resolutions(Tables T, u64 n, u64 ts_floor, const u32* set, u32 mask,
                                                                         const u64* ids, u8* slots) {
    extern __shared__ __attribute__((aligned(16))) u8 s_lds[];
    u32* s_set = (u32*)s_lds;
    for (u32 i = threadIdx.x; i <= mask; i += PENDING_THREADS) s_set[i] = set[i];
    __syncthreads();
    for (u32 t = 0; t < PENDING_TILES; t++) {
        const u64 tile0 = ((u64)blockIdx.x * PENDING_TILES + t) * PENDING_THREADS, pos = tile0 + threadIdx.x;
        if (tile0 >= n) break;
        if (pos >= n) continue;
        const ulonglong2* c = (const ulonglong2*)&T.xlog[pos];
        const ulonglong2 d = c[7];
        const u32 tf = (u32)(d.x >> 48);
        if (d.y <= ts_floor || !(tf & (TF_POST | TF_VOID)) || (tf & TF_PENDING)) continue;
        const ulonglong2 p = c[4];
        const u32 index = tb_change_probe(s_set, mask, ids, p.x, p.y);
        if (index == CHANGE_NONE) continue;
        const ulonglong2 id = c[0];
        if (tb_id_reserved(id.x, id.y) || tb_transfer_find(T, id.x, id.y) != (u32)pos) continue;
        *(Transfer*)(slots + (u64)index * 128) = T.xlog[pos];
    }
}
```

### tigerbeetle_amd/csrc/k_query.h

```cpp
#pragma once

#include <type_traits>

#include "pass.h"

#define QUERY_THREADS 256
#define QUERY_WAVES (QUERY_THREADS / 64)

struct QueryFields {
    u64 dlo, dhi, clo, chi, ts;
};

struct QueryFilter {
    typedef QueryFields Fields;
    u64 id_lo, id_hi;
    u64 ts_min, ts_max;
    u32 debits, credits;
    __device__ bool pass(const QueryFields& f) const {
        return (debits && f.dlo == id_lo && f.dhi == id_hi) || (credits && f.clo == id_lo && f.chi == id_hi);
    }
};

struct QueryFieldVals {
    u64 u128_lo, u128_hi, u64v, ts;
    u32 u32v, ledger, code;
};

struct QueryFieldFilter {
    typedef QueryFieldVals Fields;
    u64 u128_lo, u128_hi, u64v;
    u64 ts_min, ts_max;
    u32 u32v, ledger, code;
    __host__ __device__ bool wants_u128() const { return (u128_lo | u128_hi) != 0; }
    __device__ bool pass(const QueryFieldVals& f) const {
        return (!wants_u128() || (f.u128_lo == u128_lo && f.u128_hi == u128_hi)) && (!u64v || f.u64v == u64v) &&
               (!u32v || f.u32v == u32v) && (!ledger || f.ledger == ledger) && (!code || f.code == code);
    }
};

#define PENDING_OPEN (1u << 4)
#define PENDING_EXPIRED (1u << 5)
#define PENDING_POSTED (1u << 6)
#define PENDING_VOIDED (1u << 7)
#define PENDING_STATES (PENDING_OPEN | PENDING_EXPIRED | PENDING_POSTED | PENDING_VOIDED)

struct QueryPendingFields {
    u64 ts;
    u32 timeout, flags;
};

struct QueryPendingFilter {
    typedef QueryPendingFields Fields;
    u64 id_lo, id_hi;
    u64 ts_min, ts_max;
    u64 now;
    u32 debits, credits;
    u32 want;
    u8* states;
    __device__ u32 state(const QueryPendingFields& f, const u8* xposted, u64 pos) const {
        const u8 st = xposted[pos];
        if (st == POSTED_POSTED) return PENDING_POSTED;
        if (st == POSTED_VOIDED) return PENDING_VOIDED;
        if (f.timeout) {
            u64 expiry = f.ts + (u64)f.timeout * 1000000000ULL;
            if (expiry < f.ts) expiry = ~0ULL;
            if (expiry <= now) return PENDING_EXPIRED;
        }
        return PENDING_OPEN;
    }
    __device__ bool pass(const QueryPendingFields& f, const Tables& T, u64 pos) const {
        if (!(f.flags & TF_PENDING)) return false;
        if ((id_lo | id_hi) != 0) {
            const ulonglong2* c = (const ulonglong2*)&T.xlog[pos];
            bool side = false;
            if (debits) {
                const ulonglong2 d = c[1];
                side = d.x == id_lo && d.y == id_hi;
            }
            if (!side && credits) {
                const ulonglong2 cr = c[2];
                side = cr.x == id_lo && cr.y == id_hi;
            }
            if (!side) return false;
        }
        return (state(f, T.xposted, pos) & want) != 0;
    }
};

template <bool COOP, typename F>
__device__ static inline typename F::Fields tb_query_fields(const Tables& T, u64 tile0, u64 n, u64* s_raw) {
    if constexpr (std::is_same<F, QueryPendingFilter>::value) {
        static_assert(!COOP, "the pending filter has no cooperative load shape");
        QueryPendingFields v{0, 0, 0};
        const u64 pos = tile0 + threadIdx.x;
        if (pos < n) {
            const ulonglong2* c = (const ulonglong2*)&T.xlog[pos];
            const ulonglong2 b = c[6], d = c[7];
            v.timeout = (u32)(b.y >> 32), v.flags = (u32)(d.x >> 48), v.ts = d.y;
        }
        return v;
    } else if constexpr (std::is_same<F, QueryFieldFilter>::value) {
        static_assert(!COOP, "the field filter has no cooperative load shape");
        QueryFieldVals v{0, 0, 0, 0, 0, 0, 0};
        const u64 pos = tile0 + threadIdx.x;
        if (pos < n) {
            const ulonglong2* c = (const ulonglong2*)&T.xlog[pos];
            const ulonglong2 a = c[5], b = c[6], d = c[7];
            v.u128_lo = a.x, v.u128_hi = a.y, v.u64v = b.x, v.u32v = (u32)b.y;
            v.ledger = (u32)d.x, v.code = (u32)(d.x >> 32) & 0xFFFF, v.ts = d.y;
        }
        return v;
    } else {
    QueryFields f{0, 0, 0, 0, 0};
    if (!COOP) {
        const u64 pos = tile0 + threadIdx.x;
        if (pos < n) {
            const ulonglong2* c = (const ulonglong2*)&T.xlog[pos];
            const ulonglong2 d = c[1], cr = c[2];
            f.ts = ((const u64*)c)[15];
            f.dlo = d.x, f.dhi = d.y, f.clo = cr.x, f.chi = cr.y;
        }
        return f;
    }
    const u32 lane = threadIdx.x & 63, wave = threadIdx.x >> 6;
    const u64 wave0 = tile0 + (u64)wave * 64;
    ulonglong2* s = (ulonglong2*)s_raw + wave * 192;
#pragma unroll
    for (u32 j = 0; j < 3; j++) {
        const u32 idx = j * 64 + lane, r = idx / 3, q = idx % 3;
        ulonglong2 v{0, 0};
        if (wave0 + r < n) v = ((const ulonglong2*)&T.xlog[wave0 + r])[q == 2 ? 7 : q + 1];
        s[idx] = v;
    }
    __syncthreads();
    const ulonglong2 d = s[lane * 3], cr = s[lane * 3 + 1], t = s[lane * 3 + 2];
    f.dlo = d.x, f.dhi = d.y, f.clo = cr.x, f.chi = cr.y, f.ts = t.y;
    return f;
    }
}

template <typename F>
__device__ static inline bool tb_query_hit(const Tables& T, const F& flt, u64 pos, u64 n, const typename F::Fields& f) {
    if (pos >= n || f.ts == 0 || f.ts < flt.ts_min || f.ts > flt.ts_max) return false;
    if constexpr (std::is_same<F, QueryPendingFilter>::value) {
        if (!flt.pass(f, T, pos)) return false;
    } else {
        if (!flt.pass(f)) return false;
    }
    const u64* idw = (const u64*)&T.xlog[pos];
    const u64 lo = idw[0], hi = idw[1];
    if (tb_id_reserved(lo, hi)) return false;
    return tb_transfer_find(T, lo, hi) == (u32)pos;
}

template <bool COOP, typename F>
__global__ __launch_bounds__(QUERY_THREADS) void tb_query_count(Tables T, F flt, u64 n, u32* counts, u64* mins,
                                                                u64* maxs, u32* ordered) {
    __shared__ __attribute__((aligned(16))) u64 s_chunks[COOP ? QUERY_WAVES * 192 * 2 : 2];
    __shared__ u64 s_max[QUERY_WAVES], s_min[QUERY_WAVES];
    __shared__ u32 s_cnt[QUERY_WAVES], s_bad[QUERY_WAVES];
    const u64 tile0 = (u64)blockIdx.x * QUERY_THREADS;
    const u32 lane = threadIdx.x & 63, wave = threadIdx.x >> 6;
    const typename F::Fields f = tb_query_fields<COOP, F>(T, tile0, n, s_chunks);
    const bool hit = tb_query_hit(T, flt, tile0 + threadIdx.x, n, f);
    u64 incl = hit ? f.ts : 0;
#pragma unroll
    for (u32 off = 1; off < 64; off <<= 1) {
        const u64 o = __shfl_up((unsigned long long)incl, off);
        if (lane >= off && o > incl) incl = o;
    }
    u64 before = __shfl_up((unsigned long long)incl, 1);
    if (lane == 0) before = 0;
    u64 lo = hit ? f.ts : ~0ULL;
#pragma unroll
    for (u32 off = 32; off > 0; off >>= 1) {
        const u64 o = __shfl_xor((unsigned long long)lo, off);
        if (o < lo) lo = o;
    }
    const u64 m = __ballot(hit);
    if (lane == 63) s_max[wave] = incl;
    if (lane == 0) {
        s_min[wave] = lo;
        s_cnt[wave] = __popcll(m);
    }
    __syncthreads();
    for (u32 w = 0; w < wave; w++) before = max(before, s_max[w]);
    const u64 bad = __ballot(hit && f.ts <= before);
    if (lane == 0) s_bad[wave] = bad != 0;
    __syncthreads();
    if (threadIdx.x == 0) {
        u32 c = 0, b = 0;
        u64 mn = ~0ULL, mx = 0;
        for (u32 w = 0; w < QUERY_WAVES; w++) {
            c += s_cnt[w];
            b |= s_bad[w];
            mn = min(mn, s_min[w]);
            mx = max(mx, s_max[w]);
        }
        counts[blockIdx.x] = c;
        mins[blockIdx.x] = mn;
        maxs[blockIdx.x] = mx;
        ordered[blockIdx.x] = !b;
    }
}

__global__ __launch_bounds__(1024) void tb_query_scan(const u32* counts, const u64* mins, const u64* maxs, const u32* ordered,
                                                      u64 nblocks, u64* base, u64* res) {
    __shared__ u32 s_wave[1024 / 64];
    __shared__ u64 s_wmax[1024 / 64];
    const u32 lane = threadIdx.x & 63, wave = threadIdx.x >> 6;
    const u64 per = (nblocks + 1023) / 1024;
    const u64 k0 = min(nblocks, (u64)threadIdx.x * per), k1 = min(nblocks, k0 + per);
    u32 local = 0;
    u64 lmax = 0;
    for (u64 k = k0; k < k1; k++) {
        local += counts[k];
        if (counts[k]) lmax = max(lmax, maxs[k]);
    }
    u32 all;
    u64 run = tb_block_excl_sum(local, s_wave, &all);
    u64 incl = lmax;
#pragma unroll
    for (u32 off = 1; off < 64; off <<= 1) {
        const u64 o = __shfl_up((unsigned long long)incl, off);
        if (lane >= off && o > incl) incl = o;
    }
    u64 seen = __shfl_up((unsigned long long)incl, 1);
    if (lane == 0) seen = 0;
    if (lane == 63) s_wmax[wave] = incl;
    __syncthreads();
    for (u32 w = 0; w < wave; w++) seen = max(seen, s_wmax[w]);
    int bad = 0;
    for (u64 k = k0; k < k1; k++) {
        base[k] = run;
        run += counts[k];
        if (counts[k]) {
            bad |= !ordered[k] || mins[k] <= seen;
            seen = max(seen, maxs[k]);
        }
    }
    bad = __syncthreads_or(bad);
    if (threadIdx.x == 0) {
        res[0] = all;
        res[1] = !bad;
    }
}

__device__ static inline u32 tb_query_tile_rank(bool hit, u32* s_cnt) {
    const u32 lane = threadIdx.x & 63, wave = threadIdx.x >> 6;
    const u64 m = __ballot(hit);
    if (lane == 0) s_cnt[wave] = __popcll(m);
    __syncthreads();
    u32 r = __popcll(m & ((1ULL << lane) - 1));
    for (u32 w = 0; w < wave; w++) r += s_cnt[w];
    return r;
}

template <typename F>
__global__ __launch_bounds__(QUERY_THREADS) void tb_query_scatter(Tables T, F flt, u64 n, const u32* counts,
                                                                  const u64* base, const u64* res, u32 k, u32 reversed,
                                                                  u8* out) {
    __shared__ u32 s_cnt[QUERY_WAVES];
    const u64 total = res[0], b0 = base[blockIdx.x], c = counts[blockIdx.x];
    const u64 kk = min((u64)k, total), lo = reversed ? total - kk : 0, hi = lo + kk;
    if (!res[1] || c == 0 || b0 >= hi || b0 + c <= lo) return;
    const u64 pos = (u64)blockIdx.x * QUERY_THREADS + threadIdx.x;
    const typename F::Fields f = tb_query_fields<false, F>(T, (u64)blockIdx.x * QUERY_THREADS, n, nullptr);
    const bool hit = tb_query_hit(T, flt, pos, n, f);
    const u64 rank = b0 + tb_query_tile_rank(hit, s_cnt);
    if (!hit || rank < lo || rank >= hi) return;
    const u64 dst = reversed ? total - 1 - rank : rank;
    if (dst < k) {
        *(Transfer*)(out + dst * 128) = T.xlog[pos];
        if constexpr (std::is_same<F, QueryPendingFilter>::value) flt.states[dst] = (u8)flt.state(f, T.xposted, pos);
    }
}

template <typename F>
__global__ __launch_bounds__(QUERY_THREADS) void tb_query_keys(Tables T, F flt, u64 n, u64 wg0, const u32* counts,
                                                               const u64* base, u64* keys, u64 keys_cap) {
    __shared__ u32 s_cnt[QUERY_WAVES];
    const u64 b = wg0 + blockIdx.x;
    if (counts[b] == 0) return;
    const u64 pos = b * QUERY_THREADS + threadIdx.x;
    const typename F::Fields f = tb_query_fields<false, F>(T, b * QUERY_THREADS, n, nullptr);
    const bool hit = tb_query_hit(T, flt, pos, n, f);
    const u64 rank = base[b] - base[wg0] + tb_query_tile_rank(hit, s_cnt);
    if (hit && rank < keys_cap) {
        keys[2 * rank] = f.ts;
        keys[2 * rank + 1] = pos;
    }
}

__global__ __launch_bounds__(QUERY_THREADS) void tb_query_gather(Tables T, const u64* positions, u32 m, u64 n, u8* out) {
    const u32 i = blockIdx.x * QUERY_THREADS + threadIdx.x;
    if (i >= m) return;
    const u64 pos = positions[i];
    if (pos < n) *(Transfer*)(out + (u64)i * 128) = T.xlog[pos];
}
```

### tigerbeetle_amd/csrc/k_query_many.h

```cpp
#pragma once

#include "k_query.h"

#define QUERY_MANY_FILTERS 64
#define QUERY_MANY_SLOTS 128
#define QUERY_MANY_TILES 64
#define QUERY_MANY_DEPTH 4
static_assert(QUERY_MANY_TILES * QUERY_WAVES <= QUERY_THREADS, "a thread per {tile, wave} of a chunk");
static_assert(QUERY_MANY_TILES <= 64, "a chunk's tiles are one u64 of bits");

struct QueryManyTable {
    ulonglong2 id[QUERY_MANY_SLOTS];
    u64 mask[QUERY_MANY_SLOTS];
    u64 ts_min[QUERY_MANY_FILTERS], ts_max[QUERY_MANY_FILTERS];
    u32 k[QUERY_MANY_FILTERS];
    u64 debits, credits, reversed;
    u64 windows;
};
static_assert(sizeof(QueryManyTable) % 8 == 0, "copied into LDS by words");

__host__ __device__ static inline u32 tb_qm_slot(u64 lo, u64 hi) {
    return (u32)(((lo ^ (hi * 0x9E3779B97F4A7C15ULL)) * 0xD6E8FEB86659FD93ULL) >> 57) & (QUERY_MANY_SLOTS - 1);
}

// ... 165 lines not shown
                const u32 o = __shfl_up(incl, off);
                if (lane >= off) incl += o;
            }
            res[QM_RES_START + lane] = incl - m;
            if (lane == 63) res[QM_RES_RECORDS] = incl;
        }
    }
    const u64 per = (nc + 1023) / 1024;
    const u64 k0 = min(nc, (u64)threadIdx.x * per), k1 = min(nc, k0 + per);
    u64 lmax = 0;
    for (u64 k = k0; k < k1; k++) lmax = max(lmax, cmax[k]);
    u64 incl = lmax;
#pragma unroll
    for (u32 off = 1; off < 64; off <<= 1) {
        const u64 o = __shfl_up((unsigned long long)incl, off);
        if (lane >= off && o > incl) incl = o;
    }
    u64 seen = __shfl_up((unsigned long long)incl, 1);
    if (lane == 0) seen = 0;
    if (lane == 63) s_wmax[wave] = incl;
    __syncthreads();
    for (u32 w = 0; w < wave; w++) seen = max(seen, s_wmax[w]);
    int bad = 0;
    for (u64 k = k0; k < k1; k++) {
        if (cmax[k]) {
            bad |= !cord[k] || cmin[k] <= seen;
            seen = max(seen, cmax[k]);
        }
    }
    bad = __syncthreads_or(bad);
    if (threadIdx.x == 0) res[QM_RES_ORDERED] = !bad;
}

__global__ __launch_bounds__(QUERY_THREADS) void tb_qm_scatter(Tables T, const QueryManyTable* tab, u64 n, u32 tiles,
                                                               const u32* counts, const u32* base, const u64* ctiles,
                                                               const u64* res, u8* out) {
    __shared__ __attribute__((aligned(16))) QueryManyTable s_tab;
    __shared__ u64 s_lo[QUERY_MANY_FILTERS], s_hi[QUERY_MANY_FILTERS], s_total[QUERY_MANY_FILTERS], s_start[QUERY_MANY_FILTERS];
    __shared__ u32 s_w[2][QUERY_WAVES][QUERY_MANY_FILTERS];
    const u32 lane = threadIdx.x & 63, wave = threadIdx.x >> 6;
    const u64 tmask = ctiles[blockIdx.x];
    if (!res[QM_RES_ORDERED] || tmask == 0) return;
    const u64 total = res[lane], kk = min((u64)tab->k[lane], total);
    const u64 lo = ((tab->reversed >> lane) & 1) ? total - kk : 0, hi = lo + kk;
    const u32 c = counts[(u64)blockIdx.x * QUERY_MANY_FILTERS + lane];
    u64 run = base[(u64)blockIdx.x * QUERY_MANY_FILTERS + lane];
    const u64 want = tb_qm_uniform(__ballot(c != 0 && run < hi && run + c > lo));
    if (want == 0) return;
    if (wave == 0) s_lo[lane] = lo, s_hi[lane] = hi, s_total[lane] = total, s_start[lane] = res[QM_RES_START + lane];
    tb_qm_load_table(&s_tab, tab);
    __syncthreads();
    u32 it = 0;
    for (u64 r = tmask; r; r &= r - 1, it ^= 1) {
        const u64 tile0 = ((u64)blockIdx.x * tiles + (u32)__builtin_ctzll(r)) * QUERY_THREADS, pos = tile0 + threadIdx.x;
        const QueryFields f = tb_query_fields<false, QueryFilter>(T, tile0, n, nullptr);
        const u64 m = tb_qm_hit(T, &s_tab, pos, n, f) & want;
        u64 wor = 0;
        u32 mine = 0;
        if (__ballot(m != 0)) {
            wor = tb_qm_wave_or(m);
            for (u64 q = wor; q; q &= q - 1) {
                const u32 bit = __builtin_ctzll(q);
                const u32 cnt = __popcll(__ballot((m >> bit) & 1));
                if (lane == bit) mine = cnt;
            }
        }
        s_w[it][wave][lane] = mine;
        __syncthreads();
        u32 before = 0, tot = 0;
        for (u32 w = 0; w < QUERY_WAVES; w++) {
            const u32 v = s_w[it][w][lane];
            tot += v;
            if (w < wave) before += v;
        }
        for (u64 q = wor; q; q &= q - 1) {
            const u32 bit = __builtin_ctzll(q);
            const bool has = (m >> bit) & 1;
            const u64 b = __ballot(has);
            const u64 start = __shfl((unsigned long long)(run + before), (int)bit);
            if (!has) continue;
            const u64 rank = start + __popcll(b & ((1ULL << lane) - 1));
            if (rank < s_lo[bit] || rank >= s_hi[bit]) continue;
            const u64 dst = ((s_tab.reversed >> bit) & 1) ? s_total[bit] - 1 - rank : rank;
            if (dst < s_tab.k[bit]) *(Transfer*)(out + (s_start[bit] + dst) * 128) = T.xlog[pos];
        }
        run += tot;
    }
}
```

### tigerbeetle_amd/csrc/k_replay.h

```cpp
#pragma once

#include "k_resolve.h"

enum : u32 {
    UNDO_ACCOUNT_INSERT = 1, UNDO_BALANCE_UPDATE = 2, UNDO_TRANSFER_INSERT = 3, UNDO_POSTED = 4,
    UNDO_FREE_DELTA = 5,
};

struct alignas(16) UndoEntry {
    u32 kind;
    u32 slot;
    u64 pad;
    AccountBal before;
};

struct Replay {
    Tables T;
    UndoEntry* undo;
    u32 undo_len;
    u32 undo_cap;
    u64 log_base;
    bool scope;
    bool failed;
    u32 epoch;
// ... 151 lines not shown
                R.T.g->account_count--;
                break;
            case UNDO_BALANCE_UPDATE: rp_bal_store<FLOW>(R.T.bal, e.slot, e.before); break;
            case UNDO_FREE_DELTA: {
                AccountBal neg;
                neg.debits_pending = (u128)0 - e.before.debits_pending;
                neg.debits_posted = (u128)0 - e.before.debits_posted;
                neg.credits_pending = (u128)0 - e.before.credits_pending;
                neg.credits_posted = (u128)0 - e.before.credits_posted;
                rp_add_free_delta(R, e.slot, neg);
                break;
            }
            case UNDO_TRANSFER_INSERT:
                tb_xindex_tombstone(R.T, e.slot);
                if (FLOW) R.xcount--;
                else R.T.g->transfer_count--;
                break;
            case UNDO_POSTED: rp_store_posted<FLOW>(R.T, e.slot, POSTED_NONE); break;
            }
        }
    }
    R.undo_len = 0;
    R.scope = false;
}

__device__ static inline u128 rp_add(Replay& R, u128 a, u128 b) {
    u128 r;
    if (tb_add_overflows(a, b, &r)) rp_panic(R, PANIC_OVERFLOW);
    return r;
}

template <bool FLOW>
__device__ static inline AccountBal rp_balance_load(Replay& R, u32 slot, bool* free) {
    *free = FLOW && !fl_account_is_resource(R.T, slot, R.epoch, R.cert_global);
    if (*free) return AccountBal{};
    return rp_bal_load<FLOW>(R.T.bal, slot);
}

template <bool FLOW>
__device__ static inline void rp_balance_update(Replay& R, u32 slot, const AccountBal& before, const AccountBal& next) {
    if (FLOW && !fl_account_is_resource(R.T, slot, R.epoch, R.cert_global)) {
        AccountBal d;
        d.debits_pending = next.debits_pending - before.debits_pending;
        d.debits_posted = next.debits_posted - before.debits_posted;
        d.credits_pending = next.credits_pending - before.credits_pending;
        d.credits_posted = next.credits_posted - before.credits_posted;
        rp_push(R, UNDO_FREE_DELTA, slot, &d);
        rp_add_free_delta(R, slot, d);
        return;
    }
    rp_push(R, UNDO_BALANCE_UPDATE, slot, &before);
    rp_bal_store<FLOW>(R.T.bal, slot, next);
}

template <bool FLOW>
__device__ static inline void rp_transfer_insert(Replay& R, const Transfer& t, u32 log_pos) {
    rp_store<FLOW>(&R.T.xlog[log_pos], t);
    if (FLOW) asm volatile("s_waitcnt vmcnt(0)" ::: "memory");
    const u32 entry = tb_transfer_claim_new(R.T, tb_lo(t.id), tb_hi(t.id), log_pos);
    if (entry == TB_NOT_FOUND) {
        R.failed = true;
        return;
    }
    if (FLOW) R.xcount++;
    else R.T.g->transfer_count++;
    rp_push(R, UNDO_TRANSFER_INSERT, entry, nullptr);
}

template <bool FLOW>
__device__ static inline u32 rp_post_or_void(Replay& R, const Transfer& t, u32 log_pos, const FastHint* hint = nullptr) {
    const Tables& T = R.T;
    const u16 f = t.flags;
    if ((f & TF_POST) && (f & TF_VOID)) return CT_FLAGS_ARE_MUTUALLY_EXCLUSIVE;
    if (f & TF_PENDING) return CT_FLAGS_ARE_MUTUALLY_EXCLUSIVE;
    if (f & TF_BAL_DEBIT) return CT_FLAGS_ARE_MUTUALLY_EXCLUSIVE;
    if (f & TF_BAL_CREDIT) return CT_FLAGS_ARE_MUTUALLY_EXCLUSIVE;
    if (t.pending_id == 0) return CT_PENDING_ID_MUST_NOT_BE_ZERO;
    if (t.pending_id == TB_U128_MAX) return CT_PENDING_ID_MUST_NOT_BE_INT_MAX;
    if (t.pending_id == t.id) return CT_PENDING_ID_MUST_BE_DIFFERENT;
    if (t.timeout != 0) return CT_TIMEOUT_RESERVED_FOR_PENDING_TRANSFER;

    const u32 pslot = rp_transfer_find<FLOW>(T, tb_lo(t.pending_id), tb_hi(t.pending_id));
    if (pslot == TB_NOT_FOUND) return CT_PENDING_TRANSFER_NOT_FOUND;
    const Transfer p = rp_load<FLOW>(&T.xlog[pslot]);
    if (!(p.flags & TF_PENDING)) return CT_PENDING_TRANSFER_NOT_PENDING;
    const u32 drs = hint ? hint->drs : tb_account_find(T, tb_lo(p.debit_account_id), tb_hi(p.debit_account_id));
    const u32 crs = hint ? hint->crs : tb_account_find(T, tb_lo(p.credit_account_id), tb_hi(p.credit_account_id));
    if (drs == TB_NOT_FOUND || crs == TB_NOT_FOUND) {
        rp_panic(R, PANIC_ASSERT);
        return R_OK;
    }
    if (t.debit_account_id > 0 && t.debit_account_id != p.debit_account_id) {
        return CT_PENDING_TRANSFER_HAS_DIFFERENT_DEBIT_ACCOUNT_ID;
    }
    if (t.credit_account_id > 0 && t.credit_account_id != p.credit_account_id) {
        return CT_PENDING_TRANSFER_HAS_DIFFERENT_CREDIT_ACCOUNT_ID;
    }
    if (t.ledger > 0 && t.ledger != p.ledger) return CT_PENDING_TRANSFER_HAS_DIFFERENT_LEDGER;
    if (t.code > 0 && t.code != p.code) return CT_PENDING_TRANSFER_HAS_DIFFERENT_CODE;
    const u128 amount = t.amount > 0 ? t.amount : p.amount;
    if (amount > p.amount) return CT_EXCEEDS_PENDING_TRANSFER_AMOUNT;
    if ((f & TF_VOID) && amount < p.amount) return CT_PENDING_TRANSFER_HAS_DIFFERENT_AMOUNT;

    const u32 es = rp_transfer_find<FLOW>(T, tb_lo(t.id), tb_hi(t.id));
    if (es != TB_NOT_FOUND) return tb_post_void_exists(t, rp_load<FLOW>(&T.xlog[es]), p);
    const u8 posted = rp_load_posted<FLOW>(T, pslot);
    if (posted == POSTED_POSTED) return CT_PENDING_TRANSFER_ALREADY_POSTED;
    if (posted == POSTED_VOIDED) return CT_PENDING_TRANSFER_ALREADY_VOIDED;
    if (!(p.timestamp < t.timestamp)) {
        rp_panic(R, PANIC_ASSERT);
        return R_OK;
    }
    if (p.timeout > 0) {
        const u64 timeout_ns = (u64)p.timeout * 1000000000ULL;
        const u64 expiry = p.timestamp + timeout_ns;
        if (expiry < p.timestamp) {
            rp_panic(R, PANIC_OVERFLOW);
            return R_OK;
        }
        if (t.timestamp >= expiry) return CT_PENDING_TRANSFER_EXPIRED;
    }

    Transfer r;
    r.id = t.id;
    r.debit_account_id = p.debit_account_id;
    r.credit_account_id = p.credit_account_id;
    r.user_data_128 = t.user_data_128 > 0 ? t.user_data_128 : p.user_data_128;
    r.user_data_64 = t.user_data_64 > 0 ? t.user_data_64 : p.user_data_64;
    r.user_data_32 = t.user_data_32 > 0 ? t.user_data_32 : p.user_data_32;
    r.ledger = p.ledger;
    r.code = p.code;
    r.pending_id = t.pending_id;
    r.timeout = 0;
    r.timestamp = t.timestamp;
    r.flags = t.flags;
    r.amount = amount;
    rp_transfer_insert<FLOW>(R, r, log_pos);
    if (R.failed) return R_OK;

    rp_push(R, UNDO_POSTED, pslot, nullptr);
    rp_store_posted<FLOW>(T, pslot, (f & TF_POST) ? POSTED_POSTED : POSTED_VOIDED);

    bool dfree, cfree;
    const AccountBal dr0 = rp_balance_load<FLOW>(R, drs, &dfree);
    const AccountBal cr0 = rp_balance_load<FLOW>(R, crs, &cfree);
    AccountBal dr = dr0, cr = cr0;
    if ((!dfree && dr.debits_pending < p.amount) || (!cfree && cr.credits_pending < p.amount)) {
        rp_panic(R, PANIC_OVERFLOW);
        return R_OK;
    }
    dr.debits_pending -= p.amount;
    cr.credits_pending -= p.amount;
    if (f & TF_POST) {
        dr.debits_posted = rp_add(R, dr.debits_posted, amount);
        cr.credits_posted = rp_add(R, cr.credits_posted, amount);
    }
    rp_balance_update<FLOW>(R, drs, dr0, dr);
    rp_balance_update<FLOW>(R, crs, cr0, cr);
    return R_OK;
}

template <bool FLOW>
__device__ static inline u32 rp_create_transfer(Replay& R, const Transfer& t, u32 log_pos,
                                                const FastHint* hint = nullptr) {
    const Tables& T = R.T;
    const u16 f = t.flags;
    if (f & TF_PADDING) return CT_RESERVED_FLAG;
// ... 251 lines not shown
```

### tigerbeetle_amd/csrc/k_route.h

```cpp
#pragma once

#include "pass.h"

#define ROUTE_THREADS 256
#define ROUTE_WORLD_MAX 64
#define ROUTE_LOCAL 0xFF
#define SLOT_LOCAL 0xFFFFFFFFu
#define ROUTE_DEP 0xFE
#define SLOT_DEP 0xFFFFFFFEu

enum : u32 { ROUTE_DIRTY_FLAGS = 1, ROUTE_DIRTY_LIMIT = 2 };


__host__ __device__ static inline u64 tb_limit_bit(u64 lo, u64 hi, u64 mask) {
    return tb_mix64(tb_hash_id(lo, hi) ^ 0x9e3779b97f4a7c15ULL) & mask;
}
__device__ static inline bool tb_limit_maybe(const u64* bits, u64 mask, u64 lo, u64 hi) {
    if (tb_id_reserved(lo, hi)) return false;
    const u64 b = tb_limit_bit(lo, hi, mask);
    return (bits[b >> 6] >> (b & 63)) & 1;
}
__device__ static inline void tb_limit_set(u64* bits, u64 mask, u64 lo, u64 hi) {
    const u64 b = tb_limit_bit(lo, hi, mask);
    atomicOr((unsigned long long*)&bits[b >> 6], 1ULL << (b & 63));
// ... 187 lines not shown
    u32 a = 0, b = n;
    while (a < b) {
        const u32 m = (a + b) >> 1;
        const u64 mh = marked[2 * m + 1], ml = marked[2 * m];
        if (mh < hi || (mh == hi && ml < lo)) a = m + 1; else b = m;
    }
    return a < n && marked[2 * a] == lo && marked[2 * a + 1] == hi;
}

__global__ __launch_bounds__(ROUTE_THREADS) void tb_route_dependents(RouteArgs A, const u64* marked, u32 n_marked,
                                                                    u8* dep) {
    const u64 e = (u64)blockIdx.x * ROUTE_THREADS + threadIdx.x;
    if (e >= A.n) return;
    const u64* w = (const u64*)(A.events + e * 128);
    const u16 flags = *(const u16*)(A.events + e * 128 + 118);
    const u32 b = tb_batch_search(A.batch_off, 0, A.nb, e);
    u8 d = 0;
    if ((flags & TF_LINKED) || (e > A.batch_off[b] && (*(const u16*)(A.events + (e - 1) * 128 + 118) & TF_LINKED))) d |= 1;
    if (flags & (TF_POST | TF_VOID)) d |= 2;
    if (flags & (TF_BAL_DEBIT | TF_BAL_CREDIT)) d |= 4;
    if (A.T.g->limit_accounts != 0) {
        const u32 dr = tb_account_find(A.T, w[2], w[3]);
        const u32 cr = tb_account_find(A.T, w[4], w[5]);
        if ((dr != TB_NOT_FOUND && (A.T.acct_hot[dr].flags & AF_LIMITS)) ||
            (cr != TB_NOT_FOUND && (A.T.acct_hot[cr].flags & AF_LIMITS))) {
            d |= 8;
        }
    }
    if (n_marked && (tb_route_marked(marked, n_marked, w[2], w[3]) || tb_route_marked(marked, n_marked, w[4], w[5]))) {
        d |= 16;
    }
    dep[e] = d;
}

__global__ void tb_route_homes(const u64* ids, u64 n, u32 world, u8* out) {
    const u64 i = (u64)blockIdx.x * blockDim.x + threadIdx.x;
    if (i < n) out[i] = (u8)tb_home(ids[2 * i], ids[2 * i + 1], world);
}

__global__ __launch_bounds__(1024) void tb_route_replies(const u64* batch_off, const u32* slot, const u8* codes,
                                                        u32* results, u32* reply_bytes) {
    __shared__ u32 s_wave[1024 / 64];
    const u32 b = blockIdx.x;
    const u64 boff = batch_off[b];
    const u32 L = (u32)(batch_off[b + 1] - boff);
    u32* out = results + 2 * boff;
    u32 running = 0;
    for (u32 c = 0; c < L; c += blockDim.x) {
        const u32 i = c + threadIdx.x;
        u32 code = R_OK;
        if (i < L) {
            const u32 s = slot[boff + i];
            code = s == SLOT_LOCAL ? R_TIMESTAMP_MUST_BE_ZERO : codes[s];
        }
        const u64 m = __ballot(code != R_OK);
        const u32 lane = threadIdx.x & 63, wave = threadIdx.x >> 6;
        if (lane == 0) s_wave[wave] = __popcll(m);
        __syncthreads();
        u32 wb = 0, tot = 0;
        for (u32 k = 0; k < blockDim.x / 64; k++) {
            wb += k < wave ? s_wave[k] : 0;
            tot += s_wave[k];
        }
        if (code != R_OK) {
            const u32 r = running + wb + __popcll(m & ((1ULL << lane) - 1));
            out[2 * r] = i;
            out[2 * r + 1] = code;
        }
        running += tot;
        __syncthreads();
    }
    if (threadIdx.x == 0) reply_bytes[b] = running * 8;
}


__global__ void tb_fetch_transfers(Tables T, const u64* ids, u32 n, u8* out, u8* state) {
    const u32 i = blockIdx.x * blockDim.x + threadIdx.x;
    if (i >= n) return;
    const u32 pos = tb_transfer_find(T, ids[2 * i], ids[2 * i + 1]);
    if (pos == TB_NOT_FOUND) {
        state[i] = 0;
        return;
    }
    *(Transfer*)(out + (u64)i * 128) = T.xlog[pos];
    state[i] = 1 + T.xposted[pos];
}

__global__ void tb_upsert_accounts(Tables T, const u8* recs, u32 n, u32* status, u32 if_absent, BalView snap) {
    const u32 i = blockIdx.x * blockDim.x + threadIdx.x;
    if (i >= n) return;
    const Account a = *(const Account*)(recs + (u64)i * 128);
    u32 slot = tb_account_find(T, tb_lo(a.id), tb_hi(a.id));
    if (slot != TB_NOT_FOUND) {
        if (if_absent) return;
        AccountBal b;
        b.debits_pending = a.debits_pending;
        b.debits_posted = a.debits_posted;
        b.credits_pending = a.credits_pending;
        b.credits_posted = a.credits_posted;
        tb_bal_store(T.bal, slot, b);
        return;
    }
    slot = tb_account_claim(T, tb_lo(a.id), tb_hi(a.id), a.timestamp);
    if (slot == TB_NOT_FOUND) {
        atomicOr(status, 1u);
        return;
    }
    tb_account_store_new(T, slot, a);
    if (snap.lo) tb_bal_store(snap, slot, tb_bal_load(T.bal, slot));
    atomicAdd((unsigned long long*)&T.g->account_count, 1ULL);
}

__global__ void tb_upsert_transfers(Tables T, const u8* recs, const u8* state, u32 n, u64 log_base, u32* counter,
                                    u32* status, u32 if_absent, u8* snap_posted) {
    const u32 i = blockIdx.x * blockDim.x + threadIdx.x;
    if (i >= n) return;
    const Transfer& t = *(const Transfer*)(recs + (u64)i * 128);
    const u32 pos = tb_transfer_find(T, tb_lo(t.id), tb_hi(t.id));
    const u8 st = state[i];
    if (pos != TB_NOT_FOUND) {
        if (if_absent) return;
        if (st) T.xposted[pos] = st - 1;
        return;
    }
    const u64 lp = log_base + atomicAdd(counter, 1u);
    if (lp >= T.xlog_cap) {
        atomicOr(status, 1u);
        return;
    }
    T.xlog[lp] = t;
    T.xposted[lp] = st ? st - 1 : POSTED_NONE;
    if (snap_posted) snap_posted[lp] = T.xposted[lp];
    if (tb_transfer_claim_new(T, tb_lo(t.id), tb_hi(t.id), (u32)lp) == TB_NOT_FOUND) atomicOr(status, 1u);
    atomicAdd((unsigned long long*)&T.g->transfer_count, 1ULL);
}

#define OWNER_LEG_WORDS 5
#define NODE_LEG_WORDS 3

struct OwnerLegArgs {
    u32 world;
    u32 self;
    u64* legs;
    u64 cap;
    u64* counts;
    const u32* os_of;
    u32 words;
};

__global__ __launch_bounds__(256) void tb_owner_legs(PassArgs P, OwnerLegArgs O) {
    static_assert(VALIDATE_THREADS == 256, "tb_stage_events stages 256 records");
    __shared__ __attribute__((aligned(16))) u8 stage[256 * STAGE_STRIDE];
    __shared__ u32 s_cnt[ROUTE_WORLD_MAX];
    __shared__ u64 s_base[ROUTE_WORLD_MAX];
    if (threadIdx.x < O.world) s_cnt[threadIdx.x] = 0;
    const u32 tile0 = blockIdx.x * 256;
    tb_stage_events((const u8*)(P.T.xlog + P.log_base + tile0), (u32)min((u64)256, P.n - tile0), stage);
    const u32 pe = tile0 + threadIdx.x;
    u32 owner[2] = {0, 0}, pos[2] = {0, 0}, oslot[2] = {0, 0};
    bool emit[2] = {false, false};
    u128 acct[2] = {0, 0}, amount = 0;
    u32 field0 = 0;
    if (pe < P.n && P.codes[P.e0 + pe] == R_OK) {
        const u64* c1 = (const u64*)(stage + tb_stage_off(threadIdx.x, 1));
        const u64* c2 = (const u64*)(stage + tb_stage_off(threadIdx.x, 2));
        const u64* c3 = (const u64*)(stage + tb_stage_off(threadIdx.x, 3));
        const u16 flags = *(const u16*)(stage + tb_stage_off(threadIdx.x, 7) + 6);
// ... 78 lines not shown
```

### tigerbeetle_amd/csrc/k_statement.h

```cpp
#pragma once

#include "k_asof.h"

#define STATEMENT_IDS_MAX 4095u
#define STATEMENT_ROW_BYTES 256u
#define STATEMENT_ZONE1 8
#define STATEMENT_SIDE_WORDS 7
#define STATEMENT_BIN_WORDS 22
#define STATEMENT_LDS_BINS 112u
#define STATEMENT_RES_MATCHED 0
#define STATEMENT_RES_ORPHAN 1
#define STATEMENT_RES_WORDS 2

struct StatementFlows {
    u128 pending_in, pending_out, posted_in;
};
__host__ __device__ static inline StatementFlows tb_statement_flows(u32 flags, u128 amount, u128 p) {
    if (tb_effect_is_post(flags)) return {0, p, amount};
    if (flags & TF_PENDING) return {amount, 0, 0};
    if (flags & TF_VOID) return {0, amount, 0};
    return {0, 0, amount};
}

__global__ __launch_bounds__(CHANGE_THREADS) void tb_statement_effects(NodeTablesArgs N, u32 self, u64 n, u64 t_open, u64 t_close,
                                                                      const u32* set, u32 mask, const u64* ids, u32 n_ids,
                                                                      u64* bins) {
    extern __shared__ __attribute__((aligned(16))) u8 s_lds[];
    u32* s_set = (u32*)s_lds;
    u64* s_bins = (u64*)(s_set + mask + 1);
    u32* s_tags = (u32*)(s_bins + STATEMENT_LDS_BINS * STATEMENT_BIN_WORDS);
    const Tables& T = N.T[self];
    const u32 lane = threadIdx.x & 63;
    u64* flags = bins + (u64)n_ids * STATEMENT_BIN_WORDS;
    for (u32 i = threadIdx.x; i <= mask; i += CHANGE_THREADS) s_set[i] = set[i];
    for (u32 i = threadIdx.x; i < STATEMENT_LDS_BINS * STATEMENT_BIN_WORDS; i += CHANGE_THREADS) s_bins[i] = 0;
    for (u32 i = threadIdx.x; i < STATEMENT_LDS_BINS; i += CHANGE_THREADS) s_tags[i] = CHANGE_NONE;
    __syncthreads();
    for (u32 t = 0; t < CHANGE_TILES; t++) {
        const u64 tile0 = ((u64)blockIdx.x * CHANGE_TILES + t) * CHANGE_THREADS, pos = tile0 + threadIdx.x;
        if (tile0 >= n) break;
        const u64* w = (const u64*)&T.xlog[pos < n ? pos : 0];
        const u64 ts = pos < n ? w[15] : 0;
        const bool wanted = ts > t_open;
        if (__ballot(wanted) == 0) continue;
        const u32 zone = t_close != 0 && ts > t_close ? 0 : 1;
        u32 idx[2] = {CHANGE_NONE, CHANGE_NONE};
        u128 a0 = 0, a1 = 0, a2 = 0;
        if (wanted) {
            const ulonglong2 d = ((const ulonglong2*)w)[1], c = ((const ulonglong2*)w)[2];
            idx[0] = tb_change_probe(s_set, mask, ids, d.x, d.y);
            idx[1] = tb_change_probe(s_set, mask, ids, c.x, c.y);
        }
        if ((idx[0] & idx[1]) != CHANGE_NONE) {
            const u64 lo = w[0], hi = w[1];
            if (tb_id_reserved(lo, hi) || tb_transfer_find(T, lo, hi) != (u32)pos) {
                idx[0] = idx[1] = CHANGE_NONE;
            } else {
                const u128 amount = tb_u128(w[6], w[7]);
                const u32 tf = (u32)(w[14] >> 48);
                u128 p = amount;
                if (tb_effect_is_post(tf) && !tb_pending_amount(N, w[8], w[9], &p)) {
                    atomicOr((unsigned long long*)flags, 1ULL);
                }
                if (zone == 0) {
                    const BalanceEffect e = tb_balance_effect(tf, amount, p);
                    a0 = e.pend, a1 = e.post;
                } else {
                    const StatementFlows f = tb_statement_flows(tf, amount, p);
                    a0 = f.pending_in, a1 = f.pending_out, a2 = f.posted_in;
                }
            }
        }
#pragma unroll
        for (u32 side = 0; side < 2; side++) {
            const u32 index = idx[side];
            bool adds = index != CHANGE_NONE;
            const u32 my = adds ? index * 2 + zone : CHANGE_NONE;
            u128 v0 = adds ? a0 : (u128)0, v1 = adds ? a1 : (u128)0, v2 = adds ? a2 : (u128)0;
            u32 count = adds ? 1 : 0;
            u32 nxt = lane;
            bool chains = false;
            u64 todo = __ballot(adds);
            while (todo) {
                const int leader = __ffsll((unsigned long long)todo) - 1;
                const u32 b = __shfl(my, leader);
                const bool mine = my == b;
                const u64 group = __ballot(mine);
                todo &= ~group;
                if ((group & (group - 1)) == 0) continue;
                chains = true;
                if (mine) {
                    const u64 above = lane == 63 ? 0 : group & ~((2ULL << lane) - 1);
                    if (above) nxt = (u32)__ffsll((unsigned long long)above) - 1;
                    if ((int)lane != leader) adds = false;
                }
            }
            if (chains) {
#pragma unroll
                for (u32 s = 0; s < 6; s++) {
                    const bool has = nxt != lane;
                    const u128 o0 = tb_shfl128(v0, nxt), o1 = tb_shfl128(v1, nxt), o2 = tb_shfl128(v2, nxt);
                    const u32 oc = __shfl(count, nxt);
                    const u32 nn = __shfl(nxt, nxt);
                    if (has) {
                        v0 += o0, v1 += o1, v2 += o2, count += oc;
                        nxt = nn == nxt ? lane : nn;
                    }
                }
            }
            if (!adds) continue;
            const u32 at = tb_change_bin_claim(s_tags, STATEMENT_LDS_BINS, index);
            u64* bin = at != CHANGE_NONE ? s_bins + at * STATEMENT_BIN_WORDS : bins + (u64)index * STATEMENT_BIN_WORDS;
            if (zone == 0) {
                tb_atomic_add128(bin + 4 * side, v0);
                tb_atomic_add128(bin + 4 * side + 2, v1);
            } else {
                u64* dst = bin + STATEMENT_ZONE1 + STATEMENT_SIDE_WORDS * side;
                tb_atomic_add128(dst, v0);
                tb_atomic_add128(dst + 2, v1);
                tb_atomic_add128(dst + 4, v2);
                atomicAdd((unsigned long long*)(dst + 6), (unsigned long long)count);
            }
        }
    }
    __syncthreads();
// ... 74 lines not shown
```

### tigerbeetle_amd/csrc/k_validate.h

```cpp
#pragma once

#include "pass.h"

#define TB_CODE_PANIC 63u

struct TransferScratch {
    u32 hz = 0;
    u32 dr = TB_NOT_FOUND, cr = TB_NOT_FOUND;
    u32 ps = TB_NOT_FOUND;
    u32 rs = TB_NOT_FOUND;
    u128 amount = 0;
    u128 contrib = 0;
    u64 kid = 0, kpid = 0;
    u64 rec_ts = 0;
};

__device__ static inline u32 tb_transfer_exists(const Transfer& t, const Transfer& e) {
    if (t.flags != e.flags) return CT_EXISTS_WITH_DIFFERENT_FLAGS;
    if (t.debit_account_id != e.debit_account_id) return CT_EXISTS_WITH_DIFFERENT_DEBIT_ACCOUNT_ID;
    if (t.credit_account_id != e.credit_account_id) return CT_EXISTS_WITH_DIFFERENT_CREDIT_ACCOUNT_ID;
    if (t.amount != e.amount) return CT_EXISTS_WITH_DIFFERENT_AMOUNT;
    if (t.user_data_128 != e.user_data_128) return CT_EXISTS_WITH_DIFFERENT_USER_DATA_128;
    if (t.user_data_64 != e.user_data_64) return CT_EXISTS_WITH_DIFFERENT_USER_DATA_64;
    if (t.user_data_32 != e.user_data_32) return CT_EXISTS_WITH_DIFFERENT_USER_DATA_32;
// ... 16 lines not shown
        if (t.user_data_128 != e.user_data_128) return CT_EXISTS_WITH_DIFFERENT_USER_DATA_128;
    }
    if (t.user_data_64 == 0) {
        if (e.user_data_64 != p.user_data_64) return CT_EXISTS_WITH_DIFFERENT_USER_DATA_64;
    } else {
        if (t.user_data_64 != e.user_data_64) return CT_EXISTS_WITH_DIFFERENT_USER_DATA_64;
    }
    if (t.user_data_32 == 0) {
        if (e.user_data_32 != p.user_data_32) return CT_EXISTS_WITH_DIFFERENT_USER_DATA_32;
    } else {
        if (t.user_data_32 != e.user_data_32) return CT_EXISTS_WITH_DIFFERENT_USER_DATA_32;
    }
    return CT_EXISTS;
}

__device__ static inline Transfer tb_compose_post_void(const Transfer& t, const Transfer& p, u64 ts) {
    Transfer r;
    r.id = t.id;
    r.debit_account_id = p.debit_account_id;
    r.credit_account_id = p.credit_account_id;
    r.amount = t.amount > 0 ? t.amount : p.amount;
    r.pending_id = t.pending_id;
    r.user_data_128 = t.user_data_128 > 0 ? t.user_data_128 : p.user_data_128;
    r.user_data_64 = t.user_data_64 > 0 ? t.user_data_64 : p.user_data_64;
    r.user_data_32 = t.user_data_32 > 0 ? t.user_data_32 : p.user_data_32;
    r.timeout = 0;
    r.ledger = p.ledger;
    r.code = p.code;
    r.flags = t.flags;
    r.timestamp = ts;
    return r;
}

__device__ static inline u32 tb_claim_id(const PassArgs& P, const Transfer& t, u32 pe, TransferScratch& s,
                                         u32* exists_pos, u64 first = ~0ULL) {
    s.kid = tb_dedup_key(tb_lo(t.id), tb_hi(t.id));
    if (TB_ABL(P, ABL_SPEC)) return CLAIM_NEW;
    u32 entry = TB_NOT_FOUND;
    if (TB_ABL(P, ABL_CAS)) {
        s.rs = (u32)tb_xi_home(tb_lo(t.id), tb_hi(t.id), P.T.xidx_mask);
        s.hz |= HZ_SPEC;
        return CLAIM_NEW;
    }
    const u32 r = tb_transfer_claim(P.T, tb_lo(t.id), tb_hi(t.id), P.log_base + pe, P.log_base, exists_pos, &entry,
                                    first);
    if (r == CLAIM_NEW) {
        s.rs = entry;
        s.hz |= HZ_SPEC;
    } else if (r == CLAIM_COLLIDED) {
        s.hz |= HZ_SELFDEP;
        P.pass_words[PW_DUP] = 1;
    }
    return r;
}

__device__ static inline u32 tb_validate_post_void(const PassArgs& P, const Transfer& t, u64 ts, u32 pe,
                                                   TransferScratch& s) {
    const Tables& T = P.T;
    const u16 f = t.flags;
    if ((f & TF_POST) && (f & TF_VOID)) return CT_FLAGS_ARE_MUTUALLY_EXCLUSIVE;
    if (f & TF_PENDING) return CT_FLAGS_ARE_MUTUALLY_EXCLUSIVE;
    if (f & TF_BAL_DEBIT) return CT_FLAGS_ARE_MUTUALLY_EXCLUSIVE;
    if (f & TF_BAL_CREDIT) return CT_FLAGS_ARE_MUTUALLY_EXCLUSIVE;
    if (t.pending_id == 0) return CT_PENDING_ID_MUST_NOT_BE_ZERO;
    if (t.pending_id == TB_U128_MAX) return CT_PENDING_ID_MUST_NOT_BE_INT_MAX;
    if (t.pending_id == t.id) return CT_PENDING_ID_MUST_BE_DIFFERENT;
    if (t.timeout != 0) return CT_TIMEOUT_RESERVED_FOR_PENDING_TRANSFER;

    s.hz |= HZ_POSTVOID | HZ_PV_KEY;
    P.pass_words[PW_PV] = 1;
    s.kpid = tb_dedup_key(tb_lo(t.pending_id), tb_hi(t.pending_id));
    tb_dedup_mark(P);
    if (tb_dedup_insert(P.dedup, P.dedup_mask, s.kpid)) P.pass_words[PW_DUP] = 1;
    u32 es = TB_NOT_FOUND;
    const u32 claim = tb_claim_id(P, t, pe, s, &es);
    if (claim == CLAIM_COLLIDED) return R_OK;

    const u32 pslot = tb_transfer_find(T, tb_lo(t.pending_id), tb_hi(t.pending_id));
    if (pslot != TB_NOT_FOUND && (u64)pslot >= P.log_base) {
        s.hz |= HZ_SELFDEP;
        return R_OK;
    }
    if (pslot == TB_NOT_FOUND) return CT_PENDING_TRANSFER_NOT_FOUND;
    const Transfer p = T.xlog[pslot];
    if (!(p.flags & TF_PENDING)) return CT_PENDING_TRANSFER_NOT_PENDING;

    const u32 drs = tb_account_find(T, tb_lo(p.debit_account_id), tb_hi(p.debit_account_id));
    const u32 crs = tb_account_find(T, tb_lo(p.credit_account_id), tb_hi(p.credit_account_id));
    if (drs == TB_NOT_FOUND || crs == TB_NOT_FOUND) return TB_CODE_PANIC;

    if (t.debit_account_id > 0 && t.debit_account_id != p.debit_account_id) {
        return CT_PENDING_TRANSFER_HAS_DIFFERENT_DEBIT_ACCOUNT_ID;
    }
    if (t.credit_account_id > 0 && t.credit_account_id != p.credit_account_id) {
        return CT_PENDING_TRANSFER_HAS_DIFFERENT_CREDIT_ACCOUNT_ID;
    }
    if (t.ledger > 0 && t.ledger != p.ledger) return CT_PENDING_TRANSFER_HAS_DIFFERENT_LEDGER;
    if (t.code > 0 && t.code != p.code) return CT_PENDING_TRANSFER_HAS_DIFFERENT_CODE;

    const u128 amount = t.amount > 0 ? t.amount : p.amount;
    if (amount > p.amount) return CT_EXCEEDS_PENDING_TRANSFER_AMOUNT;
    if ((f & TF_VOID) && amount < p.amount) return CT_PENDING_TRANSFER_HAS_DIFFERENT_AMOUNT;

    if (claim == CLAIM_EXISTS) return tb_post_void_exists(t, T.xlog[es], p);

    const u8 posted = T.xposted[pslot];
    if (posted == POSTED_POSTED) return CT_PENDING_TRANSFER_ALREADY_POSTED;
    if (posted == POSTED_VOIDED) return CT_PENDING_TRANSFER_ALREADY_VOIDED;

    if (!(p.timestamp < ts)) return TB_CODE_PANIC;
    if (p.timeout > 0) {
        const u64 timeout_ns = (u64)p.timeout * 1000000000ULL;
        const u64 expiry = p.timestamp + timeout_ns;
        if (expiry < p.timestamp) return TB_CODE_PANIC;
        if (ts >= expiry) return CT_PENDING_TRANSFER_EXPIRED;
    }

    s.dr = drs;
    s.cr = crs;
    s.ps = pslot;
    s.hz |= HZ_ACCTS;
    if ((T.acct_hot[drs].flags | T.acct_hot[crs].flags) & AF_LIMITS) s.hz |= HZ_LIMIT;
    s.amount = (f & TF_POST) ? amount : 0;

    if ((s.hz & HZ_SPEC) && !P.inplace) T.xlog[P.log_base + pe] = tb_compose_post_void(t, p, ts);
    return R_OK;
}

__device__ static inline u32 tb_validate_transfer(const PassArgs& P, const Transfer& t, u64 ts, u32 pe,
                                                  TransferScratch& s) {
    const Tables& T = P.T;
    const u16 f = t.flags;
    if (f & TF_PADDING) return CT_RESERVED_FLAG;
    if (t.id == 0) return CT_ID_MUST_NOT_BE_ZERO;
    if (t.id == TB_U128_MAX) return CT_ID_MUST_NOT_BE_INT_MAX;

    if (f & (TF_POST | TF_VOID)) return tb_validate_post_void(P, t, ts, pe, s);

    if (t.debit_account_id == 0) return CT_DEBIT_ACCOUNT_ID_MUST_NOT_BE_ZERO;
    if (t.debit_account_id == TB_U128_MAX) return CT_DEBIT_ACCOUNT_ID_MUST_NOT_BE_INT_MAX;
    if (t.credit_account_id == 0) return CT_CREDIT_ACCOUNT_ID_MUST_NOT_BE_ZERO;
    if (t.credit_account_id == TB_U128_MAX) return CT_CREDIT_ACCOUNT_ID_MUST_NOT_BE_INT_MAX;
    if (t.credit_account_id == t.debit_account_id) return CT_ACCOUNTS_MUST_BE_DIFFERENT;
    if (t.pending_id != 0) return CT_PENDING_ID_MUST_BE_ZERO;
    if (!(f & TF_PENDING)) {
        if (t.timeout != 0) return CT_TIMEOUT_RESERVED_FOR_PENDING_TRANSFER;
    }
    if (!(f & (TF_BAL_DEBIT | TF_BAL_CREDIT))) {
        if (t.amount == 0) return CT_AMOUNT_MUST_NOT_BE_ZERO;
    }
    if (t.ledger == 0) return CT_LEDGER_MUST_NOT_BE_ZERO;
    if (t.code == 0) return CT_CODE_MUST_NOT_BE_ZERO;

    const u64 dlo = tb_lo(t.debit_account_id), dhi = tb_hi(t.debit_account_id);
    const u64 clo = tb_lo(t.credit_account_id), chi = tb_hi(t.credit_account_id);
    const u64 dpos = tb_hash_id(dlo, dhi) & T.account_mask;
    const u64 cpos = tb_hash_id(clo, chi) & T.account_mask;
    const u64 xpos = tb_xi_home(tb_lo(t.id), tb_hi(t.id), T.xidx_mask);
    const bool fake = TB_ABL(P, ABL_ACCTS);
    AccountHot d0 = {}, c0 = {};
    if (!fake) {
        d0 = T.acct_hot[dpos];
        c0 = T.acct_hot[cpos];
    }
    u64 x0 = ~0ULL;
    if (!TB_ABL(P, ABL_SPEC | ABL_CAS)) {
        x0 = tb_transfer_cas_home(T, tb_lo(t.id), tb_hi(t.id), (u32)(P.log_base + pe), xpos);
        if (x0 == 0) {
            s.rs = (u32)xpos;
            s.hz |= HZ_SPEC;
        }
    }
    AccountHot dr = {}, cr = {};
    u32 drs, crs;
    if (fake) {
        drs = (u32)(dlo & 1023);
        crs = (u32)(clo & 1023);
    } else {
        tb_account_find2(T, dlo, dhi, dpos, d0, clo, chi, cpos, c0, &drs, &crs, &dr, &cr);
    }
    u32 early = R_OK;
    if (drs == TB_NOT_FOUND) early = CT_DEBIT_ACCOUNT_NOT_FOUND;
    else if (crs == TB_NOT_FOUND) early = CT_CREDIT_ACCOUNT_NOT_FOUND;
    else if (!(ts > dr.timestamp) || !(ts > cr.timestamp)) early = TB_CODE_PANIC;
    else if (dr.ledger != cr.ledger) early = CT_ACCOUNTS_MUST_HAVE_THE_SAME_LEDGER;
    else if (t.ledger != dr.ledger) early = CT_TRANSFER_MUST_HAVE_THE_SAME_LEDGER_AS_ACCOUNTS;
    const bool balancing = (f & (TF_BAL_DEBIT | TF_BAL_CREDIT)) != 0;
    if (early == R_OK) {
        s.contrib = balancing && t.amount == 0 ? (u128)UINT64_MAX : t.amount;
        s.dr = drs;
        s.cr = crs;
        s.hz |= HZ_ACCTS;
        if ((dr.flags | cr.flags) & AF_LIMITS) s.hz |= HZ_LIMIT;
        if (balancing) {
            s.hz |= HZ_BAL;
            if (f & TF_BAL_DEBIT) P.T.account_mark[drs] = P.epoch;
            if (f & TF_BAL_CREDIT) P.T.account_mark[crs] = P.epoch;
            P.pass_words[PW_BAL] = 1;
        }
    }
    u32 es = TB_NOT_FOUND;
    const u32 claim = tb_claim_id(P, t, pe, s, &es, x0);
    if (early != R_OK) return early;
    if (claim == CLAIM_EXISTS) return tb_transfer_exists(t, T.xlog[es]);
    if (claim == CLAIM_COLLIDED || balancing) return R_OK;

    s.amount = t.amount;
    const u64 timeout_ns = (u64)t.timeout * 1000000000ULL;
    if (ts + timeout_ns < ts) return CT_OVERFLOWS_TIMEOUT;
    if ((s.hz & HZ_SPEC) && P.inplace) {
        s.hz |= HZ_INPLACE;
        P.T.xlog[P.log_base + pe].timestamp = ts;
    } else if ((s.hz & HZ_SPEC) && !TB_ABL(P, ABL_RECORD)) {
        s.rec_ts = ts;
        s.hz |= HZ_REC;
    }
    return R_OK;
}

template <bool SRC>
__global__ __launch_bounds__(VALIDATE_THREADS) void tb_transfers_validate(PassArgs P) {
    __shared__ __attribute__((aligned(16))) u8 stage[VALIDATE_THREADS * STAGE_STRIDE];

    const u32 tile0 = blockIdx.x * VALIDATE_THREADS;
    const u32 count = min((u32)VALIDATE_THREADS, P.n - tile0);
    const u32 pe = tile0 + threadIdx.x;
    const u64 e = P.e0 + pe;
    u32x4 tile[STAGE_CHUNKS];
    tb_stage_tile_issue<SRC>(P, tile0, count, tile, TB_ABL(P, EXP_NT));
    const LaneBatch B = tb_lane_batch(P, tile0, count, e, true);
    tb_stage_tile_commit<SRC>(P, tile0, count, tile, stage);

    TransferScratch s;
    if (threadIdx.x < count) {
        Transfer t = tb_read_staged<Transfer>(stage);
        const u32 L = (u32)(B.end - B.off);
        const u32 j = (u32)(e - B.off);
        u32 code;
        u64 routed_ts = 0;
        if (P.routed) {
            if (t.flags & (TF_LINKED | TF_POST | TF_VOID | TF_BAL_DEBIT | TF_BAL_CREDIT)) {
                tb_panic(P.T.g, PANIC_ASSERT);
            }
            routed_ts = t.timestamp;
            t.timestamp = 0;
        }
        if ((t.flags & TF_LINKED) && j == L - 1) {
            code = R_LINKED_EVENT_CHAIN_OPEN;
        } else if (t.timestamp != 0) {
            code = R_TIMESTAMP_MUST_BE_ZERO;
        } else {
            const u64 ts = P.routed ? routed_ts : P.ev_ts ? P.ev_ts[e] : B.ts - L + j + 1;
            code = tb_validate_transfer(P, t, ts, pe, s);
        }
        if (tb_hi(s.amount)) s.hz |= HZ_AMT_HI;
        P.info[pe] = code | s.hz;
        P.eflags[pe] = t.flags;
        P.dr[pe] = s.dr;
        P.cr[pe] = s.cr;
        if (s.hz & (HZ_POSTVOID | HZ_PV_KEY)) {
            P.ps[pe] = s.ps;
            P.kpid[pe] = s.kpid;
        }
        P.rs[pe] = s.rs;
        P.amt[pe] = tb_lo(s.amount);
        if (s.hz & HZ_AMT_HI) P.amt_hi[pe] = tb_hi(s.amount);
        if (code != R_OK) s.contrib = 0;
        if (s.rec_ts) *(u64*)(stage + tb_stage_off(threadIdx.x, 7) + 8) = s.rec_ts;
    }
    const u128 w = tb_wave_sum_u128(s.contrib);
    const u64 rec = __ballot(s.rec_ts != 0);
    const u32 lane = threadIdx.x & 63, w0 = threadIdx.x & ~63u;
    __builtin_amdgcn_fence(__ATOMIC_RELEASE, "wavefront");
    __builtin_amdgcn_wave_barrier();
    __builtin_amdgcn_fence(__ATOMIC_ACQUIRE, "wavefront");
#pragma unroll
    for (u32 r = 0; r < 8; r++) {
        const u32 c = lane + r * 64;
        const u32 row = c >> 3, part = c & 7;
        if ((rec >> row) & 1) {
            const u32x4 v = *(const u32x4*)(stage + tb_stage_off(w0 + row, part));
            u32x4* dst = (u32x4*)&P.T.xlog[P.log_base + tile0 + w0 + row] + part;
            if (TB_ABL(P, EXP_NT)) __builtin_nontemporal_store(v, dst);
            else *dst = v;
        }
    }
    __builtin_amdgcn_fence(__ATOMIC_RELEASE, "wavefront");
    __builtin_amdgcn_wave_barrier();
    if (lane == 0) {
        *(u64*)(stage + w0 * STAGE_STRIDE) = tb_lo(w);
        *(u64*)(stage + w0 * STAGE_STRIDE + 8) = tb_hi(w);
    }
    __syncthreads();
    if (threadIdx.x == 0) {
        u128 total = 0;
        for (u32 k = 0; k < VALIDATE_THREADS / 64; k++) {
            const u8* q = stage + k * 64 * STAGE_STRIDE;
            total = tb_sat_add(total, tb_u128(*(const u64*)q, *(const u64*)(q + 8)));
        }
        tb_sum_publish(P, total);
    }
}

__device__ static inline u32 tb_account_exists(const Account& a, const Account& e) {
    if (a.flags != e.flags) return CA_EXISTS_WITH_DIFFERENT_FLAGS;
    if (a.user_data_128 != e.user_data_128) return CA_EXISTS_WITH_DIFFERENT_USER_DATA_128;
    if (a.user_data_64 != e.user_data_64) return CA_EXISTS_WITH_DIFFERENT_USER_DATA_64;
    if (a.user_data_32 != e.user_data_32) return CA_EXISTS_WITH_DIFFERENT_USER_DATA_32;
    if (a.ledger != e.ledger) return CA_EXISTS_WITH_DIFFERENT_LEDGER;
    if (a.code != e.code) return CA_EXISTS_WITH_DIFFERENT_CODE;
    return CA_EXISTS;
}

__device__ static inline u32 tb_account_stateless(const Account& a) {
    if (a.reserved != 0) return CA_RESERVED_FIELD;
    if (a.flags & AF_PADDING) return CA_RESERVED_FLAG;
    if (a.id == 0) return CA_ID_MUST_NOT_BE_ZERO;
    if (a.id == TB_U128_MAX) return CA_ID_MUST_NOT_BE_INT_MAX;
    if ((a.flags & AF_DEBITS_MUST_NOT_EXCEED_CREDITS) && (a.flags & AF_CREDITS_MUST_NOT_EXCEED_DEBITS)) {
        return CA_FLAGS_ARE_MUTUALLY_EXCLUSIVE;
    }
    if (a.debits_pending != 0) return CA_DEBITS_PENDING_MUST_BE_ZERO;
    if (a.debits_posted != 0) return CA_DEBITS_POSTED_MUST_BE_ZERO;
    if (a.credits_pending != 0) return CA_CREDITS_PENDING_MUST_BE_ZERO;
    if (a.credits_posted != 0) return CA_CREDITS_POSTED_MUST_BE_ZERO;
    if (a.ledger == 0) return CA_LEDGER_MUST_NOT_BE_ZERO;
    if (a.code == 0) return CA_CODE_MUST_NOT_BE_ZERO;
    return R_OK;
}

template <bool SRC>
__global__ __launch_bounds__(VALIDATE_THREADS) void tb_accounts_validate(PassArgs P) {
    __shared__ __attribute__((aligned(16))) u8 stage[VALIDATE_THREADS * STAGE_STRIDE];
    const u32 tile0 = blockIdx.x * VALIDATE_THREADS;
    const u32 count = min((u32)VALIDATE_THREADS, P.n - tile0);
    const u32 pe = tile0 + threadIdx.x;
    const u64 e = P.e0 + pe;
    u32x4 tile[STAGE_CHUNKS];
    tb_stage_tile_issue<SRC>(P, tile0, count, tile);
    const LaneBatch B = tb_lane_batch(P, tile0, count, e, false);
    tb_stage_tile_commit<SRC>(P, tile0, count, tile, stage);
    if (threadIdx.x >= count) return;

    const Account a = tb_read_staged<Account>(stage);
    const u32 L = (u32)(B.end - B.off);
    const u32 j = (u32)(e - B.off);
    u32 code, hz = 0;
    u64 kid = 0;
    if ((a.flags & AF_LINKED) && j == L - 1) {
        code = R_LINKED_EVENT_CHAIN_OPEN;
// ... 19 lines not shown
```

### tigerbeetle_amd/csrc/pass.h

```cpp
#pragma once

#include "tb_device.h"

enum : u32 {
    HZ_KEYS = 1u << 8,
    HZ_LIMIT = 1u << 9,
    HZ_BAL = 1u << 10,
    HZ_ACCTS = 1u << 11,
    HZ_POSTVOID = 1u << 12,
    HZ_DEP = 1u << 13,
    HZ_EVAL_OK = 1u << 14,
    HZ_SPEC = 1u << 15,
    HZ_SELFDEP = 1u << 16,
    HZ_PV_KEY = 1u << 17,
    HZ_AMT_HI = 1u << 18,
    HZ_REC = 1u << 19,
    HZ_LATE = 1u << 20,
    HZ_INPLACE = 1u << 21,
};

#define SUM_SHARDS 64
#define FLOW_WORDS 16
#define VALIDATE_THREADS 256
#define RESOLVE_THREADS 1024
// ... 25 lines not shown
    u64* kpid;
    u32* dep_list;
    u32* dep_count;
    u64* dedup;
    u64 dedup_mask;
    u64* sum_shards;
    u64* pass_words;
    u64 log_base;
    Tables T;
    u32 ablate;
    u32 routed;
    u8* codes;
    u32 cert_ext;
    u32 seq_pv;
    const u64* ev_ts;
    u32 inplace;
    u32 legs;
    u32 apply_late;
    u32 late_in_flow;
    u32 leg_shift;
    u32* leg_tot;
    u32 leg_buckets;
    u32* resolve_slow;
    u64* leg_w;

    u32* leg_off;
    u32* flow_words;
    u64* kclock;
};

#define KCLOCK_ENDS 16
#define KCLOCK_LINE 16
#define KCLOCK_STRIDE (KCLOCK_LINE * (1 + KCLOCK_ENDS))
#define KCLOCK_WORDS (3 * KCLOCK_STRIDE)
__device__ static inline void tb_kclock_stamp_end(u64* kernel_words) {
    atomicMax((unsigned long long*)(kernel_words + (1 + blockIdx.x % KCLOCK_ENDS) * KCLOCK_LINE),
              (unsigned long long)wall_clock64());
}
__device__ static inline void tb_kclock_start(const PassArgs& P, u32 k) {
    if (P.kclock && blockIdx.x < 8 && threadIdx.x == 0) {
        atomicMin((unsigned long long*)(P.kclock + k * KCLOCK_STRIDE), (unsigned long long)wall_clock64());
    }
}
__device__ static inline void tb_kclock_end(const PassArgs& P, u32 k) {
    if (!P.kclock) return;
    __syncthreads();
    if (threadIdx.x == 0) tb_kclock_stamp_end(P.kclock + k * KCLOCK_STRIDE);
}

enum : u32 { CERT_EXT_U128 = 1, CERT_EXT_U64 = 2 };

#ifndef LEG_SLOTS_MAX
#define LEG_SLOTS_MAX 1024
#endif
#ifndef LEG_BUCKETS_PREF
#define LEG_BUCKETS_PREF 2048
#endif
#define LEG_BUCKETS_MAX 4096
#define LEG_PREPARES_MAX 1024
#define LEG_SPLIT_MIN 65536
#define LEGS_MIN_EVENTS (1u << 18)
#ifndef APPLY_THREADS
#define APPLY_THREADS 256
#endif
#ifndef LEG_AMT_BITS
#define LEG_AMT_BITS 52
#endif
#define LEG_AMT_MASK ((1ULL << LEG_AMT_BITS) - 1)
static_assert((1u << (64 - LEG_AMT_BITS - 2)) >= LEG_SLOTS_MAX, "leg word: slot-in-bucket field too narrow");

__device__ static inline u64 tb_event_ts(const PassArgs& P, u32 b, u64 boff, u32 L, u32 i) {
    if (P.ev_ts) return P.ev_ts[boff + i];
    return P.routed ? *(const u64*)(P.events + (boff + i) * 128 + 120) : P.batch_ts[b] - L + 1 + i;
}
__device__ static inline bool tb_ts_carried(const PassArgs& P) { return P.routed || P.ev_ts; }

#ifdef TBGPU_TIMING_KNOBS
#define TB_ABL(P, bits) ((((P).ablate) & (bits)) != 0)
#else
#define TB_ABL(P, bits) false
#endif
enum : u32 { ABL_DEDUP = 1, ABL_SPEC = 2, ABL_ACCTS = 4, ABL_XFIND = 8, ABL_STAGE = 16, ABL_RECORD = 32, ABL_CAS = 64, EXP_NT = 128,
             ABL_LEGS = 256, ABL_LEG_STORES = 512, ABL_LEG_WORK = 1024,
             ABL_FLOW = 2048 };

__device__ static inline u32 tb_batch_search(const u64* off, u32 lo, u32 hi, u64 e) {
    while (hi - lo > 1) {
        const u32 mid = (lo + hi) >> 1;
        if (off[mid] <= e) lo = mid; else hi = mid;
    }
    return lo;
}

__device__ static inline u32 tb_tile_batch(const PassArgs& P, u64 e_first, u32 count, u64 e, u32* s_range) {
    if (threadIdx.x == 0) {
        s_range[0] = tb_batch_search(P.batch_off, P.b0, P.b1, e_first);
        s_range[1] = tb_batch_search(P.batch_off, s_range[0], P.b1, e_first + count - 1) + 1;
    }
    __syncthreads();
    return tb_batch_search(P.batch_off, s_range[0], s_range[1], e);
}

__device__ static inline u32 tb_wave_batch(const u64* off, u32 lo, u32 hi, u64 tile_e0, u32 count, u64 e) {
    const u32 w0 = (u32)__builtin_amdgcn_readfirstlane(threadIdx.x >> 6) * 64;
    if (w0 >= count) return lo;
    const u64 first = tile_e0 + w0, last = tile_e0 + min(count, w0 + 64) - 1;
    const u32 a = tb_batch_search(off, lo, hi, first);
    const u32 z = tb_batch_search(off, a, hi, last) + 1;
    return tb_batch_search(off, a, z, e);
}

#define STAGE_STRIDE 128
__device__ static inline u32 tb_stage_off(u32 row, u32 chunk) { return row * STAGE_STRIDE + ((chunk ^ (row & 7)) << 4); }
typedef unsigned int u32x4 __attribute__((ext_vector_type(4)));

#define STAGE_CHUNKS 8
__device__ static inline void tb_stage_issue(const u8* src, u32 count, u32x4 (&v)[STAGE_CHUNKS], bool nt = false) {
    const u32 last = count * 8 - 1;
#pragma unroll
    for (u32 r = 0; r < STAGE_CHUNKS; r++) {
        const u32 c = min(threadIdx.x + r * VALIDATE_THREADS, last);
        const u32x4* g = (const u32x4*)(src + (u64)c * 16);
        v[r] = nt ? __builtin_nontemporal_load(g) : *g;
    }
}
__device__ static inline void tb_stage_commit(const u32x4 (&v)[STAGE_CHUNKS], u32 count, u8* lds, u8* copy = nullptr) {
#pragma unroll
    for (u32 r = 0; r < STAGE_CHUNKS; r++) {
        const u32 c = threadIdx.x + r * VALIDATE_THREADS;
        const u32 ev = c >> 3, part = c & 7;
        if (ev < count) {
            *(u32x4*)(lds + tb_stage_off(ev, part)) = v[r];
            if (copy) *(u32x4*)(copy + (u64)c * 16) = v[r];
        }
    }
    __syncthreads();
}
__device__ static inline void tb_stage_events(const u8* src, u32 count, u8* lds) {
    u32x4 v[STAGE_CHUNKS];
    tb_stage_issue(src, count, v);
    tb_stage_commit(v, count, lds);
}

template <bool SRC>
__device__ static inline void tb_stage_tile_issue(const PassArgs& P, u32 tile0, u32 count, u32x4 (&v)[STAGE_CHUNKS],
                                                  bool nt = false) {
    const u64 off = (P.e0 + tile0) * 128;
    if (SRC) tb_stage_issue(P.events_src + off, count, v);
    else tb_stage_issue(P.events + off, count, v, nt);
}
template <bool SRC>
__device__ static inline void tb_stage_tile_commit(const PassArgs& P, u32 tile0, u32 count, const u32x4 (&v)[STAGE_CHUNKS],
                                                   u8* lds) {
    tb_stage_commit(v, count, lds, SRC ? const_cast<u8*>(P.events) + (P.e0 + tile0) * 128 : nullptr);
}

struct LaneBatch {
    u64 off, end;
    u64 ts;
};
__device__ static inline LaneBatch tb_lane_batch(const PassArgs& P, u32 tile0, u32 count, u64 e, bool want_ts) {
    const u32 b = tb_wave_batch(P.batch_off, P.b0, P.b1, P.e0 + tile0, count, e);
    LaneBatch B;
    B.off = P.batch_off[b];
    B.end = P.batch_off[b + 1];
    B.ts = want_ts && !tb_ts_carried(P) ? P.batch_ts[b] : 0;
    return B;
// ... 183 lines not shown
```

### tigerbeetle_amd/csrc/tb_device.h

```cpp
#pragma once

#include <hip/hip_runtime.h>
#include <stdint.h>

typedef unsigned __int128 u128;
typedef uint64_t u64;
typedef int64_t i64;
typedef uint32_t u32;
typedef uint16_t u16;
typedef uint8_t u8;

#define TB_U128_MAX (~(u128)0)

struct alignas(16) Account {
    u128 id;
    u128 debits_pending;
    u128 debits_posted;
    u128 credits_pending;
    u128 credits_posted;
    u128 user_data_128;
    u64 user_data_64;
    u32 user_data_32;
    u32 reserved;
    u32 ledger;
// ... 117 lines not shown
    return r < a ? TB_U128_MAX : r;
}

#ifndef FL_BAR_GROUPS
#define FL_BAR_GROUPS 8
#endif
#define FL_BAR_STRIDE 32
#define FL_BAR_WORDS (FL_BAR_GROUPS + 4)
struct Globals {
    u64 commit_timestamp;
    u64 panic;
    u64 log_next;
    u64 dedup_dirty;
    u64 bound_lo, bound_hi;
    u64 dependent_total;
    u64 dependent_all;
    u64 account_count;
    u64 transfer_count;
    u64 export_count;
    u32 flow_barrier;
    u32 flow_passes;
    u64 flow_units;
    u64 flow_runs;
    u64 flow_run_units;
    u64 limit_accounts;
    u64 flow_plan_ticks;
    u64 flow_run_ticks;
    u64 bounds_passes;
    u64 bounds_units;
    u64 bounds_rounds;
    u64 bounds_skipped;
    u64 bounds_swept;
    u64 sweep_ticks[3];
    u64 flow_phase_ticks[8];
    u64 flow_exec_ticks;
    u64 walk[12];
    u64 walk_dbg[4];
    u64 sweep_u64_passes;
    u64 bounds_abandoned;
    u32 flow_bar[FL_BAR_STRIDE * FL_BAR_WORDS];
};

struct AccountHot {
    u64 id_lo, id_hi;
    u32 ledger;
    u16 code;
    u16 flags;
    u64 timestamp;
};
struct AccountBal {
    u128 debits_pending, debits_posted, credits_pending, credits_posted;
};
struct AccountCold {
    u128 user_data_128;
    u64 user_data_64;
    u32 user_data_32;
    u32 reserved;
};
static_assert(sizeof(AccountHot) == 32 && sizeof(AccountBal) == 64 && sizeof(AccountCold) == 32, "account split");

#define BAL_DP 0
#define BAL_DPOST 1
#define BAL_CP 2
#define BAL_CPOST 3
struct BalView {
    u64* lo;
    u64* hi;
};

#define XI_TOMB (1ULL << 31)
#define XI_POS_MASK 0x7FFFFFFFULL

struct Tables {
    AccountHot* acct_hot;
    BalView bal;
    AccountCold* acct_cold;
    u32* account_mark;
    u64 account_mask;
    u64* xidx;
    u8* xdup;
    u64 xidx_mask;
    Transfer* xlog;
    u8* xposted;
    u64 xlog_cap;
    Globals* g;
};

__device__ static inline void tb_panic(Globals* g, u32 code) {
    atomicOr((unsigned long long*)&g->panic, (unsigned long long)code);
}

__host__ __device__ static inline bool tb_id_reserved(u64 lo, u64 hi) {
    return (lo | hi) == 0 || (lo & hi) == ~0ULL;
}

__device__ static inline u32 tb_account_find(const Tables& T, u64 lo, u64 hi) {
    if (tb_id_reserved(lo, hi)) return TB_NOT_FOUND;
    u64 pos = tb_hash_id(lo, hi) & T.account_mask;
    for (u64 n = 0; n <= T.account_mask; n++) {
        const AccountHot* h = &T.acct_hot[pos];
        const u64 a = h->id_lo, b = h->id_hi;
        if (a == lo && b == hi) return (u32)pos;
        if ((a | b) == 0) return TB_NOT_FOUND;
        pos = (pos + 1) & T.account_mask;
    }
    return TB_NOT_FOUND;
}

__device__ static inline u32 tb_account_find_from(const Tables& T, u64 lo, u64 hi, u64 pos, const AccountHot& first,
                                                  AccountHot* hit) {
    if (first.id_lo == lo && first.id_hi == hi) {
        *hit = first;
        return (u32)pos;
    }
    if ((first.id_lo | first.id_hi) == 0 || tb_id_reserved(lo, hi)) return TB_NOT_FOUND;
    pos = (pos + 1) & T.account_mask;
    for (u64 n = 1; n <= T.account_mask; n++) {
        const AccountHot h = T.acct_hot[pos];
        if (h.id_lo == lo && h.id_hi == hi) {
            *hit = h;
            return (u32)pos;
        }
        if ((h.id_lo | h.id_hi) == 0) return TB_NOT_FOUND;
        pos = (pos + 1) & T.account_mask;
    }
    return TB_NOT_FOUND;
}

__device__ static inline void tb_account_find2(const Tables& T, u64 dlo, u64 dhi, u64 dpos, const AccountHot& d0,
                                               u64 clo, u64 chi, u64 cpos, const AccountHot& c0, u32* drs, u32* crs,
                                               AccountHot* dh, AccountHot* ch) {
    const u64 mask = T.account_mask;
    u32 ds = TB_NOT_FOUND, cs = TB_NOT_FOUND;
    bool dgo = false, cgo = false, dlate = false, clate = false;
    if (d0.id_lo == dlo && d0.id_hi == dhi) {
        ds = (u32)dpos;
        *dh = d0;
    } else {
        dgo = (d0.id_lo | d0.id_hi) != 0;
    }
    if (c0.id_lo == clo && c0.id_hi == chi) {
        cs = (u32)cpos;
        *ch = c0;
    } else {
        cgo = (c0.id_lo | c0.id_hi) != 0;
    }
    u64 dp = (dpos + 1) & mask, cp = (cpos + 1) & mask;
    for (u64 n = 0; (dgo || cgo) && n <= mask; n += 2) {
        ulonglong2 da = {0, 0}, db = {0, 0}, ca = {0, 0}, cb = {0, 0};
        const u64 dq = (dp + 1) & mask, cq = (cp + 1) & mask;
        if (dgo) {
            da = *(const ulonglong2*)&T.acct_hot[dp];
            db = *(const ulonglong2*)&T.acct_hot[dq];
        }
        if (cgo) {
            ca = *(const ulonglong2*)&T.acct_hot[cp];
            cb = *(const ulonglong2*)&T.acct_hot[cq];
        }
        if (dgo) {
            if (da.x == dlo && da.y == dhi) {
                ds = (u32)dp;
                dgo = false;
                dlate = true;
            } else if ((da.x | da.y) == 0) {
                dgo = false;
            } else if (db.x == dlo && db.y == dhi) {
// ... 78 lines not shown
__device__ static inline Account tb_account_load(const Tables& T, u32 slot) {
    const AccountHot h = T.acct_hot[slot];
    const AccountBal b = tb_bal_load(T.bal, slot);
    const AccountCold c = T.acct_cold[slot];
    Account a;
    a.id = tb_u128(h.id_lo, h.id_hi);
    a.debits_pending = b.debits_pending;
    a.debits_posted = b.debits_posted;
    a.credits_pending = b.credits_pending;
    a.credits_posted = b.credits_posted;
    a.user_data_128 = c.user_data_128;
    a.user_data_64 = c.user_data_64;
    a.user_data_32 = c.user_data_32;
    a.reserved = c.reserved;
    a.ledger = h.ledger;
    a.code = h.code;
    a.flags = h.flags;
    a.timestamp = h.timestamp;
    return a;
}

__device__ static inline void tb_account_store_new(const Tables& T, u32 slot, const Account& a) {
    AccountCold c;
    c.user_data_128 = a.user_data_128;
    c.user_data_64 = a.user_data_64;
    c.user_data_32 = a.user_data_32;
    c.reserved = a.reserved;
    T.acct_cold[slot] = c;
    AccountBal b;
    b.debits_pending = a.debits_pending;
    b.debits_posted = a.debits_posted;
    b.credits_pending = a.credits_pending;
    b.credits_posted = a.credits_posted;
    tb_bal_store(T.bal, slot, b);
    if (a.flags & AF_LIMITS) atomicAdd((unsigned long long*)&T.g->limit_accounts, 1ULL);
    AccountHot* h = &T.acct_hot[slot];
    h->ledger = a.ledger;
    h->code = a.code;
    h->flags = a.flags;
    h->id_lo = tb_lo(a.id);
    h->id_hi = tb_hi(a.id);
}

__host__ __device__ static inline u64 tb_fingerprint(u64 lo, u64 hi) {
    const u64 f = tb_mix64(hi ^ tb_mix64(lo ^ 0x6a09e667f3bcc909ULL));
    return f ? f : 1;
}

__host__ __device__ static inline u64 tb_fp32(u64 lo, u64 hi) { return (tb_fingerprint(lo, hi) >> 32) | 1; }
__device__ static inline u32 tb_xi_pos(u64 e) { return (u32)((e & XI_POS_MASK) - 1); }

#define XI_GROUP_LOG2 3
#define XI_GROUP (1ULL << XI_GROUP_LOG2)

__host__ __device__ static inline u64 tb_xi_home(u64 lo, u64 hi, u64 mask) {
    const u64 glo = (lo >> XI_GROUP_LOG2) | (hi << (64 - XI_GROUP_LOG2)), ghi = hi >> XI_GROUP_LOG2;
    const u64 h = tb_hash_id(glo, ghi);
    const u64 seg = h & (mask >> XI_GROUP_LOG2);
    const u64 rot = h >> (64 - XI_GROUP_LOG2);
    return (seg << XI_GROUP_LOG2) | ((lo + rot) & (XI_GROUP - 1));
}

__host__ __device__ static inline u64 tb_xi_next(u64 p, u64 mask) { return (p + XI_GROUP) & mask; }

__host__ __device__ static inline u64 tb_xi_steps(u64 mask) { return (mask >> XI_GROUP_LOG2) + 1; }

__device__ static inline u32 tb_transfer_find(const Tables& T, u64 lo, u64 hi) {
    if (tb_id_reserved(lo, hi)) return TB_NOT_FOUND;
    const u64 fp = tb_fp32(lo, hi);
    u64 pos = tb_xi_home(lo, hi, T.xidx_mask);
    for (u64 n = 0; n < tb_xi_steps(T.xidx_mask); n++) {
        const u64 e = T.xidx[pos];
        if (e == 0) return TB_NOT_FOUND;
        if ((e >> 32) == fp && !(e & XI_TOMB)) {
            const u32 lp = tb_xi_pos(e);
            const u64* idw = (const u64*)&T.xlog[lp];
            if (idw[0] == lo && idw[1] == hi) return lp;
        }
        pos = tb_xi_next(pos, T.xidx_mask);
    }
    return TB_NOT_FOUND;
}

enum : u32 { CLAIM_NEW = 0, CLAIM_EXISTS = 1, CLAIM_COLLIDED = 2, CLAIM_FULL = 3 };

__device__ static inline u32 tb_transfer_claim(const Tables& T, u64 lo, u64 hi, u32 log_pos, u64 pass_base,
                                               u32* found, u32* entry, u64 first = ~0ULL) {
    const u64 fp = tb_fp32(lo, hi);
    const u64 mine = (fp << 32) | ((u64)log_pos + 1);
    const u64 mask = T.xidx_mask;
    const u64 steps = tb_xi_steps(mask);
    u64 pos = tb_xi_home(lo, hi, mask);
    auto step = [&](u64 p, u64 cur) -> u32 {
        if (cur == 0) {
            cur = atomicCAS((unsigned long long*)&T.xidx[p], 0ULL, (unsigned long long)mine);
            if (cur == 0) {
                *entry = (u32)p;
                return CLAIM_NEW;
            }
        }
        if ((cur >> 32) == fp && !(cur & XI_TOMB)) {
            const u32 lp = tb_xi_pos(cur);
            if ((u64)lp >= pass_base) {
                T.xdup[p] = 1;
                return CLAIM_COLLIDED;
            }
            const u64* idw = (const u64*)&T.xlog[lp];
            if (idw[0] == lo && idw[1] == hi) {
                *found = lp;
                return CLAIM_EXISTS;
            }
        }
        return CLAIM_FULL;
    };
    u64 n = 0;
    if (first != ~0ULL) {
        if (first == 0) {
            *entry = (u32)pos;
            return CLAIM_NEW;
        }
        const u32 r = step(pos, first);
        if (r != CLAIM_FULL) return r;
        pos = tb_xi_next(pos, mask);
        n = 1;
    }
    for (; n < steps; n += 2) {
        const u64 q = tb_xi_next(pos, mask);
        const u64 e0 = *(volatile u64*)&T.xidx[pos];
        const u64 e1 = *(volatile u64*)&T.xidx[q];
        u32 r = step(pos, e0);
        if (r != CLAIM_FULL) return r;
        r = step(q, e1);
        if (r != CLAIM_FULL) return r;
        pos = tb_xi_next(q, mask);
    }
    tb_panic(T.g, PANIC_TABLE_FULL);
    return CLAIM_FULL;
}

__device__ static inline u64 tb_transfer_cas_home(const Tables& T, u64 lo, u64 hi, u32 log_pos, u64 xpos) {
    const u64 mine = (tb_fp32(lo, hi) << 32) | ((u64)log_pos + 1);
    return atomicCAS((unsigned long long*)&T.xidx[xpos], 0ULL, (unsigned long long)mine);
}

__device__ static inline u32 tb_transfer_claim_new(const Tables& T, u64 lo, u64 hi, u32 log_pos) {
    const u64 mine = (tb_fp32(lo, hi) << 32) | ((u64)log_pos + 1);
    u64 pos = tb_xi_home(lo, hi, T.xidx_mask);
    for (u64 n = 0; n < tb_xi_steps(T.xidx_mask); n++) {
        u64* e = &T.xidx[pos];
        if (*e == 0 && atomicCAS((unsigned long long*)e, 0ULL, (unsigned long long)mine) == 0ULL) return (u32)pos;
        pos = tb_xi_next(pos, T.xidx_mask);
    }
    tb_panic(T.g, PANIC_TABLE_FULL);
    return TB_NOT_FOUND;
}

__device__ static inline bool tb_transfer_claimed_in_pass(const Tables& T, u64 lo, u64 hi, u64 pass_base) {
    if (tb_id_reserved(lo, hi)) return false;
    const u64 fp = tb_fp32(lo, hi);
    u64 pos = tb_xi_home(lo, hi, T.xidx_mask);
    for (u64 n = 0; n < tb_xi_steps(T.xidx_mask); n++) {
        const u64 e = T.xidx[pos];
        if (e == 0) return false;
        if ((e >> 32) == fp && (u64)tb_xi_pos(e) >= pass_base) return true;
        pos = tb_xi_next(pos, T.xidx_mask);
    }
// ... 83 lines not shown
```

Before: 8.021 billion.

## Store in-place transfer timestamps in a separate dense side array

In the in-place speculative path, the commit timestamp is no longer written into the 128-byte transfer log record. It is written to a new u64 xts array after the pass. All readers go through tb_log_ts/tb_log_load, which fall back to xts when the record's timestamp field is zero. The aim is to avoid a scattered partial write into the wide log line during validation and to make timestamp stores dense. The cost is an extra array to allocate, clear, copy on eviction, and consult on many query paths, plus a possible correctness risk wherever a raw xlog read was not converted.

```diff
diff --git a/tigerbeetle_amd/csrc/engine.hip b/tigerbeetle_amd/csrc/engine.hip
--- a/tigerbeetle_amd/csrc/engine.hip
+++ b/tigerbeetle_amd/csrc/engine.hip
@@ -412,6 +412,7 @@
     HIPCK(hipMemsetAsync(E->T.xidx, 0, E->xidx_cap * sizeof(u64), E->stream));
     HIPCK(hipMemsetAsync(E->T.xdup, 0, E->xidx_cap, E->stream));
     HIPCK(hipMemsetAsync(E->T.xposted, 0, E->xlog_cap, E->stream));
+    HIPCK(hipMemsetAsync(E->T.xts, 0, E->xlog_cap * sizeof(u64), E->stream));
     HIPCK(hipMemsetAsync(E->bloom, 0, (E->bloom_mask + 1) / 8, E->stream));
     E->log_next = 0;
     E->evicted_total = 0;
@@ -601,7 +602,7 @@
 
     size_t free_b = 0, total_b = 0;
     HIPCK(hipMemGetInfo(&free_b, &total_b));
-    const u64 need = E->account_cap * (sizeof(Account) + 4) + E->xlog_cap * (sizeof(Transfer) + 1) +
+    const u64 need = E->account_cap * (sizeof(Account) + 4) + E->xlog_cap * (sizeof(Transfer) + 1 + sizeof(u64)) +
                      E->xidx_cap * (sizeof(u64) + 1) +
                      (u64)E->pe_max * (4 * 4 + 8 * 4 + 128 * PIPE_SLOTS + 8 + 4) + E->dedup_cap * 8;
     if (need > free_b) {
@@ -618,6 +619,7 @@
     HIPCK(tbMalloc(E->own, &E->T.xdup, E->xidx_cap));
     HIPCK(tbMalloc(E->own, &E->T.xlog, E->xlog_cap * sizeof(Transfer)));
     HIPCK(tbMalloc(E->own, &E->T.xposted, E->xlog_cap));
+    HIPCK(tbMalloc(E->own, &E->T.xts, E->xlog_cap * sizeof(u64)));
     HIPCK(tbMalloc(E->own, &E->g, sizeof(Globals)));
     {
         const u64 bits = std::min<u64>(1ULL << 34, pow2_at_least(std::max<u64>(1ULL << 16, 8 * E->xlog_cap)));
@@ -2962,9 +2964,11 @@
         const u64 m = std::min<u64>(cut, kept - a);
         HIPCK(hipMemcpyAsync(E->T.xlog + a, E->T.xlog + cut + a, m * sizeof(Transfer), hipMemcpyDeviceToDevice, E->stream));
         HIPCK(hipMemcpyAsync(E->T.xposted + a, E->T.xposted + cut + a, m, hipMemcpyDeviceToDevice, E->stream));
+        HIPCK(hipMemcpyAsync(E->T.xts + a, E->T.xts + cut + a, m * sizeof(u64), hipMemcpyDeviceToDevice, E->stream));
     }
     HIPCK(hipMemsetAsync(E->T.xlog + kept, 0, cut * sizeof(Transfer), E->stream));
     HIPCK(hipMemsetAsync(E->T.xposted + kept, 0, cut, E->stream));
+    HIPCK(hipMemsetAsync(E->T.xts + kept, 0, cut * sizeof(u64), E->stream));
     HIPCK(hipMemsetAsync(E->T.xidx, 0, E->xidx_cap * sizeof(u64), E->stream));
     if (kept) {
         hipLaunchKernelGGL(tb_evict_reindex, dim3((u32)std::min<u64>(4096, (kept + 255) / 256)), dim3(256), 0, E->stream,
diff --git a/tigerbeetle_amd/csrc/k_aux.h b/tigerbeetle_amd/csrc/k_aux.h
--- a/tigerbeetle_amd/csrc/k_aux.h
+++ b/tigerbeetle_amd/csrc/k_aux.h
@@ -14,7 +14,7 @@
     } else {
         const u32 pos = tb_transfer_find(T, lo, hi);
         found[i] = pos != TB_NOT_FOUND;
-        if (pos != TB_NOT_FOUND) *(Transfer*)(out + (u64)i * 128) = T.xlog[pos];
+        if (pos != TB_NOT_FOUND) *(Transfer*)(out + (u64)i * 128) = tb_log_load(T, pos);
     }
 }
 
@@ -34,7 +34,7 @@
     const u64 e = T.xidx[i];
     if (e == 0 || (e & XI_TOMB)) return;
     const u32 pos = tb_xi_pos(e);
-    const Transfer& t = T.xlog[pos];
+    const Transfer t = tb_log_load(T, pos);
     const u64 k = atomicAdd((unsigned long long*)count, 1ULL);
     *(Transfer*)(out + k * 128) = t;
     const u8 st = T.xposted[pos];
@@ -101,7 +101,7 @@
 
 __device__ static inline bool tb_delta_live(const Tables& T, u64 pos, u64 ts0) {
     const Transfer& t = T.xlog[pos];
-    return t.timestamp > ts0 && tb_transfer_find(T, tb_lo(t.id), tb_hi(t.id)) == (u32)pos;
+    return tb_log_ts(T, pos, t.timestamp) > ts0 && tb_transfer_find(T, tb_lo(t.id), tb_hi(t.id)) == (u32)pos;
 }
 
 __global__ __launch_bounds__(DELTA_THREADS) void tb_delta_log_count(Tables T, u64 pos0, u64 n, u64 ts0, u32* block_counts) {
@@ -130,7 +130,7 @@
     if (!live) return;
     u64 k = block_base[blockIdx.x] + __popcll(m & ((1ULL << lane) - 1));
     for (u32 w = 0; w < wave; w++) k += s_wave[w];
-    const Transfer& t = T.xlog[pos0 + i];
+    const Transfer t = tb_log_load(T, pos0 + i);
     if (out) *(Transfer*)(out + k * 128) = t;
     if (ids) {
         ids[4 * k] = tb_lo(t.debit_account_id);
@@ -169,7 +169,7 @@
         atomicOr((unsigned long long*)status, 1ULL);
         return;
     }
-    pairs[2 * q] = T.xlog[pos].timestamp;
+    pairs[2 * q] = tb_log_ts(T, pos, T.xlog[pos].timestamp);
     pairs[2 * q + 1] = pv[3 * q + 2];
 }
 
diff --git a/tigerbeetle_amd/csrc/k_change_events.h b/tigerbeetle_amd/csrc/k_change_events.h
--- a/tigerbeetle_amd/csrc/k_change_events.h
+++ b/tigerbeetle_amd/csrc/k_change_events.h
@@ -117,7 +117,7 @@
         const u64 tile0 = ((u64)blockIdx.x * CHANGE_TILES + t) * CHANGE_THREADS, pos = tile0 + threadIdx.x;
         if (tile0 >= n) break;
         const u64* w = (const u64*)&T.xlog[pos < n ? pos : 0];
-        const u64 ts = pos < n ? w[15] : 0;
+        const u64 ts = pos < n ? tb_log_ts(T, pos, w[15]) : 0;
         const bool newer = ts > t_last;
         if (__ballot(newer) == 0) continue;
         u32 idx[2] = {CHANGE_NONE, CHANGE_NONE};
diff --git a/tigerbeetle_amd/csrc/k_evict.h b/tigerbeetle_amd/csrc/k_evict.h
--- a/tigerbeetle_amd/csrc/k_evict.h
+++ b/tigerbeetle_amd/csrc/k_evict.h
@@ -30,7 +30,7 @@
     for (u64 pos = (u64)blockIdx.x * blockDim.x + threadIdx.x; pos < n; pos += (u64)gridDim.x * blockDim.x) {
         const Transfer& t = T.xlog[pos];
         const u64 lo = tb_lo(t.id), hi = tb_hi(t.id);
-        const bool alive = t.timestamp != 0 && !tb_id_reserved(lo, hi) && tb_transfer_find(T, lo, hi) == (u32)pos;
+        const bool alive = tb_log_ts(T, pos, t.timestamp) != 0 && !tb_id_reserved(lo, hi) && tb_transfer_find(T, lo, hi) == (u32)pos;
         if (pos < cut) {
             if (alive) {
                 tb_bloom_add(bloom, mask, lo, hi);
diff --git a/tigerbeetle_amd/csrc/k_ledgers.h b/tigerbeetle_amd/csrc/k_ledgers.h
--- a/tigerbeetle_amd/csrc/k_ledgers.h
+++ b/tigerbeetle_amd/csrc/k_ledgers.h
@@ -179,7 +179,7 @@
         const u64 tile0 = ((u64)blockIdx.x * LEDGER_LOG_TILES + t) * LEDGER_THREADS, pos = tile0 + threadIdx.x;
         if (tile0 >= n) break;
         const u64* w = (const u64*)&T.xlog[pos < n ? pos : 0];
-        const u64 ts = pos < n ? w[15] : 0;
+        const u64 ts = pos < n ? tb_log_ts(T, pos, w[15]) : 0;
         const bool newer = ts > t_at;
         if (__ballot(newer) == 0) continue;
         u32 my = CHANGE_NONE;
diff --git a/tigerbeetle_amd/csrc/k_node.h b/tigerbeetle_amd/csrc/k_node.h
--- a/tigerbeetle_amd/csrc/k_node.h
+++ b/tigerbeetle_amd/csrc/k_node.h
@@ -677,7 +677,7 @@
         const Tables& H = N.T[tb_home(q.lo, q.hi, N.world)];
         const u32 pos = tb_transfer_find(H, q.lo, q.hi);
         if (pos == TB_NOT_FOUND) continue;
-        const Transfer t = H.xlog[pos];
+        const Transfer t = tb_log_load(H, pos);
         const u32 xp = (u32)tb_wave_claim(true, loaded);
         X.xlog[xp] = t;
         X.xposted[xp] = H.xposted[pos];
@@ -740,7 +740,7 @@
                                            u64 h_base, u64* h_count) {
     const u64 stride = (u64)gridDim.x * blockDim.x;
     for (u64 i = (u64)blockIdx.x * blockDim.x + threadIdx.x; i < n; i += stride) {
-        const Transfer& t = X.xlog[base + i];
+        const Transfer t = tb_log_load(X, base + i);
         if (t.timestamp == 0 || tb_home(tb_lo(t.id), tb_hi(t.id), world) != self) continue;
         if (tb_transfer_find(X, tb_lo(t.id), tb_hi(t.id)) != (u32)(base + i)) continue;
         const u64 lp = h_base + tb_wave_claim(true, h_count);
diff --git a/tigerbeetle_amd/csrc/k_pending.h b/tigerbeetle_amd/csrc/k_pending.h
--- a/tigerbeetle_amd/csrc/k_pending.h
+++ b/tigerbeetle_amd/csrc/k_pending.h
@@ -14,8 +14,8 @@
     if (pos >= n) return;
     const ulonglong2* c = (const ulonglong2*)&T.xlog[pos];
     const ulonglong2 b = c[6], d = c[7];
-    const QueryPendingFields f{d.y, (u32)(b.y >> 32), (u32)(d.x >> 48)};
-    *(Transfer*)(out + (u64)i * 128) = T.xlog[pos];
+    const QueryPendingFields f{tb_log_ts(T, pos, d.y), (u32)(b.y >> 32), (u32)(d.x >> 48)};
+    *(Transfer*)(out + (u64)i * 128) = tb_log_load(T, pos);
     flt.states[i] = (u8)flt.state(f, T.xposted, pos);
 }
 
@@ -32,12 +32,12 @@
         const ulonglong2* c = (const ulonglong2*)&T.xlog[pos];
         const ulonglong2 d = c[7];
         const u32 tf = (u32)(d.x >> 48);
-        if (d.y <= ts_floor || !(tf & (TF_POST | TF_VOID)) || (tf & TF_PENDING)) continue;
+        if (!(tf & (TF_POST | TF_VOID)) || (tf & TF_PENDING) || tb_log_ts(T, pos, d.y) <= ts_floor) continue;
         const ulonglong2 p = c[4];
         const u32 index = tb_change_probe(s_set, mask, ids, p.x, p.y);
         if (index == CHANGE_NONE) continue;
         const ulonglong2 id = c[0];
         if (tb_id_reserved(id.x, id.y) || tb_transfer_find(T, id.x, id.y) != (u32)pos) continue;
-        *(Transfer*)(slots + (u64)index * 128) = T.xlog[pos];
+        *(Transfer*)(slots + (u64)index * 128) = tb_log_load(T, pos);
     }
 }
diff --git a/tigerbeetle_amd/csrc/k_query.h b/tigerbeetle_amd/csrc/k_query.h
--- a/tigerbeetle_amd/csrc/k_query.h
+++ b/tigerbeetle_amd/csrc/k_query.h
@@ -96,7 +96,7 @@
         if (pos < n) {
             const ulonglong2* c = (const ulonglong2*)&T.xlog[pos];
             const ulonglong2 b = c[6], d = c[7];
-            v.timeout = (u32)(b.y >> 32), v.flags = (u32)(d.x >> 48), v.ts = d.y;
+            v.timeout = (u32)(b.y >> 32), v.flags = (u32)(d.x >> 48), v.ts = tb_log_ts(T, pos, d.y);
         }
         return v;
     } else if constexpr (std::is_same<F, QueryFieldFilter>::value) {
@@ -107,7 +107,7 @@
             const ulonglong2* c = (const ulonglong2*)&T.xlog[pos];
             const ulonglong2 a = c[5], b = c[6], d = c[7];
             v.u128_lo = a.x, v.u128_hi = a.y, v.u64v = b.x, v.u32v = (u32)b.y;
-            v.ledger = (u32)d.x, v.code = (u32)(d.x >> 32) & 0xFFFF, v.ts = d.y;
+            v.ledger = (u32)d.x, v.code = (u32)(d.x >> 32) & 0xFFFF, v.ts = tb_log_ts(T, pos, d.y);
         }
         return v;
     } else {
@@ -117,7 +117,7 @@
         if (pos < n) {
             const ulonglong2* c = (const ulonglong2*)&T.xlog[pos];
             const ulonglong2 d = c[1], cr = c[2];
-            f.ts = ((const u64*)c)[15];
+            f.ts = tb_log_ts(T, pos, ((const u64*)c)[15]);
             f.dlo = d.x, f.dhi = d.y, f.clo = cr.x, f.chi = cr.y;
         }
         return f;
@@ -135,6 +135,7 @@
     __syncthreads();
     const ulonglong2 d = s[lane * 3], cr = s[lane * 3 + 1], t = s[lane * 3 + 2];
     f.dlo = d.x, f.dhi = d.y, f.clo = cr.x, f.chi = cr.y, f.ts = t.y;
+    if (f.ts == 0 && wave0 + lane < n) f.ts = T.xts[wave0 + lane];
     return f;
     }
 }
@@ -271,7 +272,7 @@
     if (!hit || rank < lo || rank >= hi) return;
     const u64 dst = reversed ? total - 1 - rank : rank;
     if (dst < k) {
-        *(Transfer*)(out + dst * 128) = T.xlog[pos];
+        *(Transfer*)(out + dst * 128) = tb_log_load(T, pos);
         if constexpr (std::is_same<F, QueryPendingFilter>::value) flt.states[dst] = (u8)flt.state(f, T.xposted, pos);
     }
 }
@@ -296,5 +297,5 @@
     const u32 i = blockIdx.x * QUERY_THREADS + threadIdx.x;
     if (i >= m) return;
     const u64 pos = positions[i];
-    if (pos < n) *(Transfer*)(out + (u64)i * 128) = T.xlog[pos];
-}
+    if (pos < n) *(Transfer*)(out + (u64)i * 128) = tb_log_load(T, pos);
+}
diff --git a/tigerbeetle_amd/csrc/k_query_many.h b/tigerbeetle_amd/csrc/k_query_many.h
--- a/tigerbeetle_amd/csrc/k_query_many.h
+++ b/tigerbeetle_amd/csrc/k_query_many.h
@@ -271,7 +271,7 @@
             const u64 rank = start + __popcll(b & ((1ULL << lane) - 1));
             if (rank < s_lo[bit] || rank >= s_hi[bit]) continue;
             const u64 dst = ((s_tab.reversed >> bit) & 1) ? s_total[bit] - 1 - rank : rank;
-            if (dst < s_tab.k[bit]) *(Transfer*)(out + (s_start[bit] + dst) * 128) = T.xlog[pos];
+            if (dst < s_tab.k[bit]) *(Transfer*)(out + (s_start[bit] + dst) * 128) = tb_log_load(T, pos);
         }
         run += tot;
     }
diff --git a/tigerbeetle_amd/csrc/k_replay.h b/tigerbeetle_amd/csrc/k_replay.h
--- a/tigerbeetle_amd/csrc/k_replay.h
+++ b/tigerbeetle_amd/csrc/k_replay.h
@@ -257,7 +257,8 @@
 
     const u32 pslot = rp_transfer_find<FLOW>(T, tb_lo(t.pending_id), tb_hi(t.pending_id));
     if (pslot == TB_NOT_FOUND) return CT_PENDING_TRANSFER_NOT_FOUND;
-    const Transfer p = rp_load<FLOW>(&T.xlog[pslot]);
+    Transfer p = rp_load<FLOW>(&T.xlog[pslot]);
+    p.timestamp = tb_log_ts(T, pslot, p.timestamp);
     if (!(p.flags & TF_PENDING)) return CT_PENDING_TRANSFER_NOT_PENDING;
     const u32 drs = hint ? hint->drs : tb_account_find(T, tb_lo(p.debit_account_id), tb_hi(p.debit_account_id));
     const u32 crs = hint ? hint->crs : tb_account_find(T, tb_lo(p.credit_account_id), tb_hi(p.credit_account_id));
diff --git a/tigerbeetle_amd/csrc/k_route.h b/tigerbeetle_amd/csrc/k_route.h
--- a/tigerbeetle_amd/csrc/k_route.h
+++ b/tigerbeetle_amd/csrc/k_route.h
@@ -293,7 +293,7 @@
         state[i] = 0;
         return;
     }
-    *(Transfer*)(out + (u64)i * 128) = T.xlog[pos];
+    *(Transfer*)(out + (u64)i * 128) = tb_log_load(T, pos);
     state[i] = 1 + T.xposted[pos];
 }
 
diff --git a/tigerbeetle_amd/csrc/k_statement.h b/tigerbeetle_amd/csrc/k_statement.h
--- a/tigerbeetle_amd/csrc/k_statement.h
+++ b/tigerbeetle_amd/csrc/k_statement.h
@@ -40,7 +40,7 @@
         const u64 tile0 = ((u64)blockIdx.x * CHANGE_TILES + t) * CHANGE_THREADS, pos = tile0 + threadIdx.x;
         if (tile0 >= n) break;
         const u64* w = (const u64*)&T.xlog[pos < n ? pos : 0];
-        const u64 ts = pos < n ? w[15] : 0;
+        const u64 ts = pos < n ? tb_log_ts(T, pos, w[15]) : 0;
         const bool wanted = ts > t_open;
         if (__ballot(wanted) == 0) continue;
         const u32 zone = t_close != 0 && ts > t_close ? 0 : 1;
diff --git a/tigerbeetle_amd/csrc/k_validate.h b/tigerbeetle_amd/csrc/k_validate.h
--- a/tigerbeetle_amd/csrc/k_validate.h
+++ b/tigerbeetle_amd/csrc/k_validate.h
@@ -122,7 +122,7 @@
         return R_OK;
     }
     if (pslot == TB_NOT_FOUND) return CT_PENDING_TRANSFER_NOT_FOUND;
-    const Transfer p = T.xlog[pslot];
+    const Transfer p = tb_log_load(T, pslot);
     if (!(p.flags & TF_PENDING)) return CT_PENDING_TRANSFER_NOT_PENDING;
 
     const u32 drs = tb_account_find(T, tb_lo(p.debit_account_id), tb_hi(p.debit_account_id));
@@ -250,7 +250,7 @@
     if (ts + timeout_ns < ts) return CT_OVERFLOWS_TIMEOUT;
     if ((s.hz & HZ_SPEC) && P.inplace) {
         s.hz |= HZ_INPLACE;
-        P.T.xlog[P.log_base + pe].timestamp = ts;
+        s.rec_ts = ts;
     } else if ((s.hz & HZ_SPEC) && !TB_ABL(P, ABL_RECORD)) {
         s.rec_ts = ts;
         s.hz |= HZ_REC;
@@ -306,6 +306,10 @@
         P.amt[pe] = tb_lo(s.amount);
         if (s.hz & HZ_AMT_HI) P.amt_hi[pe] = tb_hi(s.amount);
         if (code != R_OK) s.contrib = 0;
+        if (P.inplace) {
+            if (!TB_ABL(P, ABL_STAMP)) P.T.xts[P.log_base + pe] = s.rec_ts;
+            s.rec_ts = 0;
+        }
         if (s.rec_ts) *(u64*)(stage + tb_stage_off(threadIdx.x, 7) + 8) = s.rec_ts;
     }
     const u128 w = tb_wave_sum_u128(s.contrib);
diff --git a/tigerbeetle_amd/csrc/pass.h b/tigerbeetle_amd/csrc/pass.h
--- a/tigerbeetle_amd/csrc/pass.h
+++ b/tigerbeetle_amd/csrc/pass.h
@@ -131,7 +131,8 @@
 #endif
 enum : u32 { ABL_DEDUP = 1, ABL_SPEC = 2, ABL_ACCTS = 4, ABL_XFIND = 8, ABL_STAGE = 16, ABL_RECORD = 32, ABL_CAS = 64, EXP_NT = 128,
              ABL_LEGS = 256, ABL_LEG_STORES = 512, ABL_LEG_WORK = 1024,
-             ABL_FLOW = 2048 };
+             ABL_FLOW = 2048,
+             ABL_STAMP = 4096 };
 
 __device__ static inline u32 tb_batch_search(const u64* off, u32 lo, u32 hi, u64 e) {
     while (hi - lo > 1) {
diff --git a/tigerbeetle_amd/csrc/tb_device.h b/tigerbeetle_amd/csrc/tb_device.h
--- a/tigerbeetle_amd/csrc/tb_device.h
+++ b/tigerbeetle_amd/csrc/tb_device.h
@@ -223,6 +223,7 @@
     u64 xidx_mask;
     Transfer* xlog;
     u8* xposted;
+    u64* xts;
     u64 xlog_cap;
     Globals* g;
 };
@@ -467,6 +468,13 @@
     return TB_NOT_FOUND;
 }
 
+__device__ static inline u64 tb_log_ts(const Tables& T, u64 pos, u64 field) { return field ? field : T.xts[pos]; }
+__device__ static inline Transfer tb_log_load(const Tables& T, u64 pos) {
+    Transfer t = T.xlog[pos];
+    t.timestamp = tb_log_ts(T, pos, t.timestamp);
+    return t;
+}
+
 enum : u32 { CLAIM_NEW = 0, CLAIM_EXISTS = 1, CLAIM_COLLIDED = 2, CLAIM_FULL = 3 };
 
 __device__ static inline u32 tb_transfer_claim(const Tables& T, u64 lo, u64 hi, u32 log_pos, u64 pass_base,
```

Result: faster. 9.085 billion (median of 6 runs) (+13.3%).
